# SilentView/EMCID

Hardware: AMD Instinct MI355X
Metric: concept-edits/sec (1 000-concept batch, SD-v1.4) (higher is better)
Workload: dtype f32 forward (2 x fp16 split MFMA, fp32 accumulate) + f64 solve

## Files before the change

emcid_amd/csrc/clip_layers.hip:

```cpp
#include "common.h"

#include <algorithm>

namespace emcid {

__global__ __launch_bounds__(256) void gather_rows16_kernel(const unsigned char* __restrict__ src, int64_t src_stride,
                                                             const int* __restrict__ idx, unsigned char* __restrict__ dst,
                                                             int64_t dst_stride, int row_bytes) {
    typedef unsigned int v4u __attribute__((ext_vector_type(4)));
    const int64_t r = blockIdx.x;
    const v4u* s = reinterpret_cast<const v4u*>(src + (int64_t)idx[r] * src_stride);
    v4u* d = reinterpret_cast<v4u*>(dst + r * dst_stride);
    for (int i = threadIdx.x; i < row_bytes / 16; i += 256) d[i] = s[i];
}

__global__ __launch_bounds__(256) void gather_f32_kernel(const float* __restrict__ src, const int* __restrict__ idx,
                                                          float* __restrict__ dst, int n) {
    const int i = blockIdx.x * 256 + threadIdx.x;
    if (i < n) dst[i] = src[idx[i]];
}

__device__ __forceinline__ unsigned long long fp_mix(unsigned long long x) {
    x ^= x >> 30; x *= 0xBF58476D1CE4E5B9ull; x ^= x >> 27; x *= 0x94D049BB133111EBull; x ^= x >> 31;
    return x;
}

__device__ __forceinline__ unsigned long long fingerprint_of(const unsigned char* data, long long bytes, unsigned long long* lds) {
    typedef unsigned long long v2u64 __attribute__((ext_vector_type(2)));
    const long long nvec = bytes / 16, ns = nvec < 4096 ? nvec : 4096;
    unsigned long long h = 0;
    v2u64 x[16];
#pragma unroll
    for (int u = 0; u < 16; ++u) {
        const long long i = threadIdx.x + 256 * u;
        const long long v = ns == nvec ? i : i * nvec / ns;
        x[u] = i < ns ? *reinterpret_cast<const v2u64*>(data + 16 * v) : (v2u64){0ull, 0ull};
    }
#pragma unroll
    for (int u = 0; u < 16; ++u) {
        const long long i = threadIdx.x + 256 * u;
        if (i < ns)
            h ^= fp_mix(x[u][0] + 0x9E3779B97F4A7C15ull * (unsigned long long)(2 * i + 1)) ^ fp_mix(x[u][1] + 0x9E3779B97F4A7C15ull * (unsigned long long)(2 * i + 2));
    }
#pragma unroll
    for (int o = 32; o > 0; o >>= 1) {
        const unsigned lo = __shfl_xor((unsigned)(h & 0xffffffffu), o, 64), hi = __shfl_xor((unsigned)(h >> 32), o, 64);
        h ^= ((unsigned long long)hi << 32) | lo;
    }
    if ((threadIdx.x & 63) == 0) lds[threadIdx.x >> 6] = h;
    __syncthreads();
    return lds[0] ^ lds[1] ^ lds[2] ^ lds[3];
}

struct FpBatch { const unsigned char* data[32]; long long bytes[32]; long long slot[32]; };

__global__ __launch_bounds__(256) void fingerprint_store_kernel(FpBatch b, long long* table) {
    __shared__ unsigned long long lds[4];
    const unsigned char* data = b.data[blockIdx.x];
    const long long bytes = b.bytes[blockIdx.x];
    const unsigned long long h = fingerprint_of(data, bytes, lds);
    if (threadIdx.x == 0) {
        long long* e = table + 4 * b.slot[blockIdx.x];
        e[0] = (long long)reinterpret_cast<uintptr_t>(data); e[1] = bytes; e[2] = (long long)h; e[3] = 0;
    }
}

__global__ __launch_bounds__(256) void fingerprint_content_kernel(FpBatch b, unsigned long long* out) {
    __shared__ unsigned long long lds[4];
    const unsigned long long h = fingerprint_of(b.data[blockIdx.x], b.bytes[blockIdx.x], lds);
    if (threadIdx.x == 0) out[b.slot[blockIdx.x]] = h;
}

struct FpSkip { unsigned long long m[4]; };

__global__ __launch_bounds__(256) void fingerprint_check_kernel(const long long* table, long long first_slot, FpSkip skip, int* flag) {
    __shared__ unsigned long long lds[4];
    if ((skip.m[blockIdx.x >> 6] >> (blockIdx.x & 63)) & 1ull) return;
    const long long* e = table + 4 * (first_slot + blockIdx.x);
    const long long bytes = e[1];
    if (bytes <= 0) return;
    const unsigned long long h = fingerprint_of(reinterpret_cast<const unsigned char*>((uintptr_t)e[0]), bytes, lds);
    if (threadIdx.x == 0 && h != (unsigned long long)e[2]) atomicOr(flag, 1);
}

struct ClipWs {
    float* qkv;
    float* mid;
    uint32_t* ctx_p;
    float* ctx_s;
    uint32_t* z_p;
    float* z_s;
    float* f_scale;
    uint32_t* f_p;
    uint32_t* xq_p;
    float* xq_s;
    float* hs_q;
};

inline int64_t clip_ws_bytes(int64_t rows, int64_t h, int64_t d) {
    const int64_t r = round_up(rows, 64);
    return 4 * (r * 3 * h + r * h + r * h + r + r * h + r + 2 * r + r * d + r * h + r + r * h) + 16 * 16;
}

inline bool clip_ws_carve(void* base, int64_t bytes, int64_t rows, int64_t h, int64_t d, ClipWs& w) {
    if (base == nullptr || !aligned16(base) || bytes < clip_ws_bytes(rows, h, d)) return false;
    const int64_t r = round_up(rows, 64);
    char* p = (char*)base;
    auto take = [&](int64_t n4) { char* q = p; p += round_up(4 * n4, 16); return q; };
    w.qkv = (float*)take(r * 3 * h);
    w.mid = (float*)take(r * h);
    w.ctx_p = (uint32_t*)take(r * h);
    w.ctx_s = (float*)take(r);
    w.z_p = (uint32_t*)take(r * h);
    w.z_s = (float*)take(r);
    w.f_scale = (float*)take(2 * r);
    w.f_p = (uint32_t*)take(r * d);
    w.xq_p = (uint32_t*)take(r * h);
    w.xq_s = (float*)take(r);
    w.hs_q = (float*)take(r * h);
    return true;
}

}

using namespace emcid;

extern "C" {

int emcid_fingerprint_store(int64_t n, const void* const* data, const int64_t* bytes, const int64_t* slots, void* table,
                            int64_t table_slots, void* stream) {
    EMCID_CHECK_ARG(n >= 0 && table && (n == 0 || (data && bytes && slots)));
    for (int64_t i0 = 0; i0 < n; i0 += 32) {
        FpBatch b{};
        const int cnt = (int)std::min<int64_t>(32, n - i0);
        for (int i = 0; i < cnt; ++i) {
            EMCID_CHECK_ARG(data[i0 + i] && bytes[i0 + i] > 0 && bytes[i0 + i] % 16 == 0 && aligned16(data[i0 + i]) &&
                            slots[i0 + i] >= 0 && slots[i0 + i] < table_slots);
            b.data[i] = (const unsigned char*)data[i0 + i]; b.bytes[i] = bytes[i0 + i]; b.slot[i] = slots[i0 + i];
        }
        hipLaunchKernelGGL(fingerprint_store_kernel, dim3((unsigned)cnt), dim3(256), 0, (hipStream_t)stream, b, (long long*)table);
    }
    EMCID_CHECK_LAUNCH();
    return EMCID_OK;
}

int emcid_fingerprint_check(const void* table, int64_t table_slots, int64_t first_slot, int64_t n_slots, const uint64_t* skip_mask,
                            int* flag, void* stream) {
    EMCID_CHECK_ARG(table && flag && first_slot >= 0 && n_slots >= 0 && first_slot + n_slots <= table_slots && n_slots <= 256);
    if (n_slots == 0) return EMCID_OK;
    FpSkip skip{};
    if (skip_mask != nullptr)
        for (int w = 0; w < 4; ++w) skip.m[w] = skip_mask[w];
    hipLaunchKernelGGL(fingerprint_check_kernel, dim3((unsigned)n_slots), dim3(256), 0, (hipStream_t)stream, (const long long*)table,
                       (long long)first_slot, skip, flag);
    EMCID_CHECK_LAUNCH();
    return EMCID_OK;
}

int emcid_fingerprint_content(int64_t n, const void* const* data, const int64_t* bytes, uint64_t* out_dev, void* stream) {
    EMCID_CHECK_ARG(n >= 0 && (n == 0 || (data && bytes && out_dev)));
    if (n == 0) return EMCID_OK;
    for (int64_t i = 0; i < n; ++i)
        EMCID_CHECK_ARG(data[i] && bytes[i] > 0 && bytes[i] % 16 == 0 && aligned16(data[i]));
    for (int64_t i0 = 0; i0 < n; i0 += 32) {
        FpBatch b{};
        const int cnt = (int)std::min<int64_t>(32, n - i0);
        for (int i = 0; i < cnt; ++i) {
            b.data[i] = (const unsigned char*)data[i0 + i]; b.bytes[i] = bytes[i0 + i]; b.slot[i] = i0 + i;
        }
        hipLaunchKernelGGL(fingerprint_content_kernel, dim3((unsigned)cnt), dim3(256), 0, (hipStream_t)stream, b,
                           (unsigned long long*)out_dev);
    }
    EMCID_CHECK_LAUNCH();
    return EMCID_OK;
}

int64_t emcid_clip_workspace_bytes(int64_t rows, int64_t h, int64_t d) { return clip_ws_bytes(rows, h, d); }

int emcid_clip_layer_head_sp16(const emcid_clip_layer_sp16* L, int64_t rows, int64_t h, int64_t d, int64_t heads, float attn_scale,
                               const int* anc, int64_t anc_ld, const int* depth, const int* rows_sel, int64_t n_sel,
                               const float* hs, const void* x_planes, const float* x_inv_scale, float* mid, void* f_planes,
                               float* f_scale, float* f_f32, void* workspace, int64_t workspace_bytes, void* stream) {
    EMCID_CHECK_ARG(L && rows > 0 && h > 0 && d > 0 && heads > 0 && h % heads == 0 && anc && depth && hs && x_planes && x_inv_scale);
    EMCID_CHECK_ARG(mid && f_planes && f_scale && n_sel > 0 && n_sel <= rows && (rows_sel != nullptr || n_sel == rows) && h % 32 == 0 && d % 32 == 0);
    ClipWs w;
    if (!clip_ws_carve(workspace, workspace_bytes, rows, h, d, w)) return fail(EMCID_ERR_BAD_ARG, __func__, "workspace too small or misaligned");
    hipStream_t st = (hipStream_t)stream;
    const int64_t D = h / heads;
    const float* q;
    int64_t ldq;
    const float* res;
    if (rows_sel == nullptr) {
        EMCID_TRY(emcid_linear_sp16_f32(x_planes, h, x_inv_scale, L->qkv_planes, h, L->qkv_inv_scale, L->qkv_bias, nullptr, 0, w.qkv,
                                        3 * h, nullptr, 0, nullptr, rows, 3 * h, h, 0, -1, stream));
        q = w.qkv, ldq = 3 * h, res = hs;
    } else {
        EMCID_TRY(emcid_linear_sp16_f32(x_planes, h, x_inv_scale, (const uint32_t*)L->qkv_planes + h * h, h, L->qkv_inv_scale + h,
                                        L->qkv_bias ? L->qkv_bias + h : nullptr, nullptr, 0, w.qkv + h, 3 * h, nullptr, 0, nullptr,
                                        rows, 2 * h, h, 0, -1, stream));
        {
            ScopedProf sp(KC_MISC, st);
            hipLaunchKernelGGL(gather_rows16_kernel, dim3((unsigned)n_sel), dim3(256), 0, st, (const unsigned char*)x_planes, 4 * h,
                               rows_sel, (unsigned char*)w.xq_p, 4 * h, (int)(4 * h));
            hipLaunchKernelGGL(gather_f32_kernel, dim3((unsigned)((n_sel + 255) / 256)), dim3(256), 0, st, x_inv_scale, rows_sel,
                               w.xq_s, (int)n_sel);
            hipLaunchKernelGGL(gather_rows16_kernel, dim3((unsigned)n_sel), dim3(256), 0, st, (const unsigned char*)hs, 4 * h,
                               rows_sel, (unsigned char*)w.hs_q, 4 * h, (int)(4 * h));
            EMCID_CHECK_LAUNCH();
        }
        EMCID_TRY(emcid_linear_sp16_f32(w.xq_p, h, w.xq_s, L->qkv_planes, h, L->qkv_inv_scale, L->qkv_bias, nullptr, 0, w.mid, h,
                                        nullptr, 0, nullptr, n_sel, h, h, 0, -1, stream));
        q = w.mid, ldq = h, res = w.hs_q;
    }
    EMCID_TRY(emcid_tree_attention_sp16(q, ldq, w.qkv + h, w.qkv + 2 * h, 3 * h, anc, anc_ld, depth, rows_sel, n_sel, heads, D,
                                        attn_scale, w.ctx_p, h, w.ctx_s, stream));
    EMCID_TRY(emcid_linear_sp16_f32(w.ctx_p, h, w.ctx_s, L->out_planes, h, L->out_inv_scale, L->out_bias, res, h, mid, h, nullptr,
                                    0, nullptr, n_sel, h, h, 0, -1, stream));
    EMCID_TRY(emcid_add_layernorm_sp16(mid, h, nullptr, 0, L->ln2_gamma, L->ln2_beta, L->ln2_eps, n_sel, h, nullptr, nullptr, w.z_p,
                                       h, w.z_s, L->fc1_bound, f_scale, stream));
    EMCID_TRY(emcid_linear_sp16_f32(w.z_p, h, w.z_s, L->fc1_planes, h, L->fc1_inv_scale, L->fc1_bias, nullptr, 0, f_f32, d,
                                    f_planes, d, f_scale, n_sel, d, h, L->act, -1, stream));
    return EMCID_OK;
}

int emcid_clip_layer_tail_sp16(const emcid_clip_layer_sp16* L, int64_t n, int64_t h, int64_t d, const void* f_planes,
                               const float* f_inv_scale, const float* mid, float* hs_out, const float* next_ln_gamma,
                               const float* next_ln_beta, float next_ln_eps, void* x_planes, float* x_inv_scale, void* stream) {
    EMCID_CHECK_ARG(L && n > 0 && h % 32 == 0 && d % 32 == 0 && f_planes && f_inv_scale && mid && hs_out);
    EMCID_TRY(emcid_linear_sp16_f32(f_planes, d, f_inv_scale, L->fc2_planes, d, L->fc2_inv_scale, L->fc2_bias, mid, h, hs_out, h,
                                    nullptr, 0, nullptr, n, h, d, 0, -1, stream));
    if (next_ln_gamma != nullptr) {
        EMCID_CHECK_ARG(next_ln_beta && x_planes && x_inv_scale);
        EMCID_TRY(emcid_add_layernorm_sp16(hs_out, h, nullptr, 0, next_ln_gamma, next_ln_beta, next_ln_eps, n, h, nullptr, nullptr,
                                           x_planes, h, x_inv_scale, nullptr, nullptr, stream));
    }
    return EMCID_OK;
}

int emcid_clip_edit_layer_tail_sp16(const emcid_clip_layer_sp16* L, int64_t n_rows, int64_t h, int64_t d, const float* f_f32,
                                    const void* f_planes, const float* f_inv_scale, const float* mid, const int64_t* lookup,
                                    const int64_t* seg, int64_t B, int64_t N, const float* zs_t, double edit_weight,
                                    int layers_left, double lam_ratio, const void* cov_factor_ws, int64_t n_layers,
                                    int64_t layer_index, int use_inverse, const float* W0, float* W, float* dW, float* K_out,
                                    float* Zc_out, void* k_planes, float* k_inv_scale, void* dual_ws, int64_t dual_ws_bytes,
                                    int* info_dev, void* linear_ws, int64_t linear_ws_bytes, float* hs_out,
                                    const float* next_ln_gamma, const float* next_ln_beta, float next_ln_eps, void* x_planes,
                                    float* x_inv_scale, void* stream) {
    EMCID_CHECK_ARG(L && n_rows > 0 && h % 32 == 0 && d % 32 == 0 && f_f32 && lookup && seg && B > 0 && N > 0 && zs_t);
    EMCID_CHECK_ARG(cov_factor_ws && W0 && W && K_out && Zc_out && dual_ws && info_dev && (hs_out == nullptr || (f_planes && f_inv_scale && mid)));
    EMCID_TRY(emcid_gather_mean_f32(f_f32, B, n_rows, d, 0, d, lookup, seg, N, K_out, d, stream));
    EMCID_CHECK_ARG((k_planes == nullptr) == (k_inv_scale == nullptr));
    if (k_planes != nullptr) {
        EMCID_TRY(emcid_split_rows_f16(K_out, d, N, d, k_planes, d, k_inv_scale, nullptr, stream));
        EMCID_TRY(emcid_linear_sp16_f32(k_planes, d, k_inv_scale, L->fc2_planes, d, L->fc2_inv_scale, L->fc2_bias, nullptr, 0, Zc_out, h,
                                        nullptr, 0, nullptr, N, h, d, 0, -1, stream));
    } else {
        EMCID_TRY(emcid_linear_ws_f32(K_out, d, W, d, L->fc2_bias, nullptr, 0, Zc_out, h, N, h, d, 0, -1, linear_ws, linear_ws_bytes, stream));
    }
    EMCID_TRY(emcid_edit_dual_apply_stage1_f64(K_out, Zc_out, zs_t, N, d, h, edit_weight, layers_left, lam_ratio, cov_factor_ws,
                                               n_layers, layer_index, 0, N, use_inverse, dual_ws, dual_ws_bytes, stream));
    EMCID_TRY(emcid_edit_dual_apply_stage2_f64(N, d, h, cov_factor_ws, n_layers, layer_index, use_inverse, 0, W0, W, dW, dual_ws,
                                               dual_ws_bytes, info_dev, stream));
    if (hs_out != nullptr) {
        EMCID_TRY(emcid_split_rows_f16(W, d, h, d, const_cast<void*>(L->fc2_planes), d, const_cast<float*>(L->fc2_inv_scale), nullptr,
                                       stream));
        EMCID_TRY(emcid_clip_layer_tail_sp16(L, n_rows, h, d, f_planes, f_inv_scale, mid, hs_out, next_ln_gamma, next_ln_beta,
                                             next_ln_eps, x_planes, x_inv_scale, stream));
    }
    return EMCID_OK;
}

int emcid_clip_layers_sp16(const emcid_clip_layer_sp16* layers, int64_t n_layers, int64_t rows, int64_t h, int64_t d, int64_t heads,
                           float attn_scale, const int* anc, int64_t anc_ld, const int* depth, float* hs, void* x_planes,
                           float* x_inv_scale, const float* next_ln_gamma, const float* next_ln_beta, float next_ln_eps,
                           void* workspace, int64_t workspace_bytes, void* stream) {
    EMCID_CHECK_ARG(layers && n_layers > 0 && hs && x_planes && x_inv_scale);
    ClipWs w;
    if (!clip_ws_carve(workspace, workspace_bytes, rows, h, d, w)) return fail(EMCID_ERR_BAD_ARG, __func__, "workspace too small or misaligned");
    for (int64_t i = 0; i < n_layers; ++i) {
        const emcid_clip_layer_sp16* L = layers + i;
        EMCID_TRY(emcid_clip_layer_head_sp16(L, rows, h, d, heads, attn_scale, anc, anc_ld, depth, nullptr, rows, hs, x_planes,
                                             x_inv_scale, w.mid, w.f_p, w.f_scale, nullptr, workspace, workspace_bytes, stream));
        const bool last = i + 1 == n_layers;
        const float* g = last ? next_ln_gamma : layers[i + 1].ln1_gamma;
        const float* b = last ? next_ln_beta : layers[i + 1].ln1_beta;
        const float eps = last ? next_ln_eps : layers[i + 1].ln1_eps;
        EMCID_TRY(emcid_clip_layer_tail_sp16(L, rows, h, d, w.f_p, w.f_scale + rows, w.mid, hs, g, b, eps, x_planes, x_inv_scale, stream));
    }
    return EMCID_OK;
}

}
```

emcid_amd/csrc/gemm_sp16.hip:

```cpp
#include "common.h"
#include "sp16.h"

#include <algorithm>

namespace emcid {

typedef _Float16 v8h __attribute__((ext_vector_type(8)));
typedef _Float16 v4h __attribute__((ext_vector_type(4)));
typedef float v16f __attribute__((ext_vector_type(16)));
typedef float v4f __attribute__((ext_vector_type(4)));
typedef unsigned int v4u __attribute__((ext_vector_type(4)));

#ifndef SP16_ONE_SLOT
#define SP16_ONE_SLOT 0
#endif
constexpr int SPK = 32;

enum SpAct : int { SP_ACT_NONE = 0, SP_ACT_QUICK_GELU = 1, SP_ACT_GELU_ERF = 2 };

template <int V> struct SpIC { static constexpr int value = V; };

__device__ __forceinline__ bool sp_al16(const void* p) { return (reinterpret_cast<uintptr_t>(p) & 15) == 0; }

struct SpArgs {
    const uint32_t* X; int64_t ldx; const float* xs;
    const uint32_t* W; int64_t ldw; const float* ws;
    const float* bias;
    const float* res; int64_t ldr;
    float* Y; int64_t ldy;
    uint32_t* P; int64_t ldp; const float* ps;
    int M, N, K, act, tiles_n, tiles, rb;
    long long* stamps;
};

__device__ __forceinline__ void sp_tile_of(const SpArgs& a, int tile, int& bm, int& bn) {
    const int tiles_m = a.tiles / a.tiles_n, sr = tile / (a.rb * a.tiles_n), rem = tile - sr * a.rb * a.tiles_n;
    const int rows = min(a.rb, tiles_m - sr * a.rb);
    bn = rem / rows;
    bm = sr * a.rb + (rem - bn * rows);
}

template <int MJ, int NI, int WM, int WN, int PF, int KS>
struct SpGeom {
    static constexpr int NW = WM * WN;
    static constexpr int NT = 64 * NW * KS;
    static constexpr int BM = 32 * MJ * WM, BN = 32 * NI * WN;
    static constexpr int PPR = 8 * KS;
    static constexpr int SBK = SPK * KS;
    static constexpr int ROW = 128 * KS + 16;
    static constexpr int VA = (BM * PPR + NT - 1) / NT, VB = (BN * PPR + NT - 1) / NT;
    static constexpr int STAGE = (BM + BN) * ROW;
    static constexpr int NBLK = MJ * NI, HB = KS == 2 ? (NBLK + 1) / 2 : NBLK;
    static constexpr int RED = KS == 2 ? NW * NBLK * 4 * 64 * 16 : 0;
    static constexpr int SMEM = 2 * STAGE > RED ? 2 * STAGE : RED;
};

template <int MJ, int NI, int WM, int WN, int PF, int DBG, int KS>
__device__ __forceinline__ void sp_accumulate(const SpArgs& a, int m0, int n0, int T, unsigned char* smem, v16f (&acc)[NI][MJ]) {
    using G = SpGeom<MJ, NI, WM, WN, PF, KS>;
    constexpr int NT = G::NT, BM = G::BM, BN = G::BN, VA = G::VA, VB = G::VB, STAGE = G::STAGE, PPR = G::PPR, SPROW = G::ROW,
                  SBK = G::SBK;
    const int tid = threadIdx.x, lane = tid & 63, wave = (tid >> 6) % G::NW, grp = (tid >> 6) / G::NW;
    const int l31 = lane & 31, l5 = lane >> 5;
    const int wm0 = (wave / WN) * (32 * MJ), wn0 = (wave % WN) * (32 * NI);

    const uint32_t* pa[VA];
    const uint32_t* pb[VB];
    int wa[VA], wb[VB];
#pragma unroll
    for (int s = 0; s < VA; ++s) {
        const int v = tid + NT * s, row = min(v / PPR, BM - 1);
        pa[s] = a.X + (int64_t)min(m0 + row, a.M - 1) * a.ldx + 4 * (v % PPR);
        wa[s] = row * SPROW + 16 * (v % PPR);
    }
#pragma unroll
    for (int s = 0; s < VB; ++s) {
        const int v = tid + NT * s, row = min(v / PPR, BN - 1);
        pb[s] = a.W + (int64_t)min(n0 + row, a.N - 1) * a.ldw + 4 * (v % PPR);
        wb[s] = (BM + row) * SPROW + 16 * (v % PPR);
    }
    constexpr bool TAIL_A = (BM * PPR) % NT != 0, TAIL_B = (BN * PPR) % NT != 0;
    const bool last_a = !TAIL_A || tid + NT * (VA - 1) < BM * PPR;
    const bool last_b = !TAIL_B || tid + NT * (VB - 1) < BN * PPR;

    v4u ga[PF][VA], gb[PF][VB];
    auto gload = [&](int it, auto rc) __attribute__((always_inline)) {
        constexpr int R = decltype(rc)::value;
        const int k0 = it * SBK;
#pragma unroll
        for (int s = 0; s < VA; ++s)
            if (s + 1 < VA || last_a) ga[R][s] = *reinterpret_cast<const v4u*>(pa[s] + k0);
#pragma unroll
        for (int s = 0; s < VB; ++s)
            if (s + 1 < VB || last_b) gb[R][s] = *reinterpret_cast<const v4u*>(pb[s] + k0);
    };
    auto lstore = [&](unsigned char* stage, auto rc) __attribute__((always_inline)) {
        constexpr int R = decltype(rc)::value;
#pragma unroll
        for (int s = 0; s < VA; ++s)
            if (s + 1 < VA || last_a) *reinterpret_cast<v4u*>(stage + wa[s]) = ga[R][s];
#pragma unroll
        for (int s = 0; s < VB; ++s)
            if (s + 1 < VB || last_b) *reinterpret_cast<v4u*>(stage + wb[s]) = gb[R][s];
    };

    const int fx_off = (wm0 + l31) * SPROW + 32 * l5 + 128 * grp;
    const int fw_off = (BM + wn0 + l31) * SPROW + 32 * l5 + 128 * grp;
    constexpr int NSLOT = ((MJ * NI > 4 && SP16_ONE_SLOT) || MJ * NI > 5) ? 1 : 2;
    v8h xh[NSLOT][MJ], xl[NSLOT][MJ], wh[NSLOT][NI], wl[NSLOT][NI];
    auto fread = [&](const unsigned char* stage, int t, int slot) __attribute__((always_inline)) {
#pragma unroll
        for (int j = 0; j < MJ; ++j) {
            xh[slot][j] = *reinterpret_cast<const v8h*>(stage + fx_off + j * 32 * SPROW + 64 * t);
            xl[slot][j] = *reinterpret_cast<const v8h*>(stage + fx_off + j * 32 * SPROW + 64 * t + 16);
        }
#pragma unroll
        for (int i = 0; i < NI; ++i) {
            wh[slot][i] = *reinterpret_cast<const v8h*>(stage + fw_off + i * 32 * SPROW + 64 * t);
            wl[slot][i] = *reinterpret_cast<const v8h*>(stage + fw_off + i * 32 * SPROW + 64 * t + 16);
        }
    };
    auto mfmas = [&](int slot, int p_lo, int p_hi) __attribute__((always_inline)) {
#pragma unroll
        for (int p = 0; p < 3; ++p)
            if (p >= p_lo && p < p_hi)
#pragma unroll
                for (int i = 0; i < NI; ++i)
#pragma unroll
                    for (int j = 0; j < MJ; ++j)
                        acc[i][j] = __builtin_amdgcn_mfma_f32_32x32x16_f16(p == 0 ? wl[slot][i] : wh[slot][i],
                                                                           p == 1 ? xl[slot][j] : xh[slot][j], acc[i][j], 0, 0, 0);
    };

    gload(0, SpIC<0>{});
    lstore(smem, SpIC<0>{});
    gload(min(1, T - 1), SpIC<1 % PF>{});
    if constexpr (PF > 1) gload(min(2, T - 1), SpIC<2 % PF>{});
    __syncthreads();
    constexpr bool ONE_SLOT = (MJ * NI > 4 && SP16_ONE_SLOT) || MJ * NI > 5;
    if constexpr (!ONE_SLOT) fread(smem, 0, 0);
    if constexpr (DBG >= 3) fread(smem, 1, 1);
    auto body = [&](auto rc, int it) __attribute__((always_inline)) {
        unsigned char* cur = smem + (it & 1) * STAGE;
        unsigned char* oth = smem + ((it + 1) & 1) * STAGE;
        if constexpr (ONE_SLOT) {
            fread(cur, 0, 0);
            mfmas(0, 0, 3);
            __builtin_amdgcn_sched_barrier(0);
            fread(cur, 1, 0);
            lstore(oth, rc);
            __syncthreads();
            gload(min(it + 1 + PF, T - 1), rc);
            __builtin_amdgcn_sched_barrier(0);
            mfmas(0, 0, 3);
            return;
        }
        __builtin_amdgcn_sched_barrier(0);
        mfmas(0, 0, 1);
        __builtin_amdgcn_sched_barrier(0);
        if constexpr (DBG < 3) fread(cur, 1, 1);
        __builtin_amdgcn_sched_barrier(0);
        mfmas(0, 1, 3);
        __builtin_amdgcn_sched_barrier(0);
        if constexpr (DBG < 2) lstore(oth, rc);
        __syncthreads();
        if constexpr (DBG < 1) gload(min(it + 1 + PF, T - 1), rc);
        __builtin_amdgcn_sched_barrier(0);
        mfmas(1, 0, 1);
        __builtin_amdgcn_sched_barrier(0);
        if constexpr (DBG < 3) fread(oth, 0, 0);
        __builtin_amdgcn_sched_barrier(0);
        mfmas(1, 1, 3);
    };
    if constexpr (PF == 1) {
        for (int it = 0; it < T; ++it) body(SpIC<0>{}, it);
    } else {
        int it = 0;
        for (; it + 1 < T; it += 2) {
            body(SpIC<1>{}, it);
            body(SpIC<0>{}, it + 1);
        }
        if (it < T) body(SpIC<1>{}, it);
    }
}

template <int MJ, int NI, int WM, int WN, int KS>
__device__ __forceinline__ void sp_finish(const SpArgs& a, int m0, int n0, unsigned char* smem, v16f (&acc)[NI][MJ]) {
    constexpr int BM = 32 * MJ * WM, BN = 32 * NI * WN, NW = WM * WN, NBLK = MJ * NI, HB = KS == 2 ? (NBLK + 1) / 2 : NBLK;
    const int tid = threadIdx.x, lane = tid & 63, wave = (tid >> 6) % NW, grp = (tid >> 6) / NW;
    const int l31 = lane & 31, l5 = lane >> 5;
    const int wm0 = (wave / WN) * (32 * MJ), wn0 = (wave % WN) * (32 * NI);
    if constexpr (KS == 2) {
        __syncthreads();
        v4f* red = reinterpret_cast<v4f*>(smem) + wave * (NBLK * 4 * 64) + lane;
        auto put = [&](auto tc) __attribute__((always_inline)) {
            constexpr int t = decltype(tc)::value;
#pragma unroll
            for (int q = 0; q < 4; ++q) {
                v4f v = {acc[t / MJ][t % MJ][4 * q], acc[t / MJ][t % MJ][4 * q + 1], acc[t / MJ][t % MJ][4 * q + 2],
                         acc[t / MJ][t % MJ][4 * q + 3]};
                red[(t * 4 + q) * 64] = v;
            }
        };
        auto take = [&](auto tc, auto first) __attribute__((always_inline)) {
            constexpr int t = decltype(tc)::value;
#pragma unroll
            for (int q = 0; q < 4; ++q) {
                const v4f v = red[(t * 4 + q) * 64];
#pragma unroll
                for (int e = 0; e < 4; ++e) {
                    const float c = acc[t / MJ][t % MJ][4 * q + e];
                    acc[t / MJ][t % MJ][4 * q + e] = decltype(first)::value ? c + v[e] : v[e] + c;
                }
            }
        };
        static_assert(NBLK <= 8, "blocks per wave");
        if (grp == 1) {
            if constexpr (0 < HB) put(SpIC<0>{});
            if constexpr (1 < HB) put(SpIC<1>{});
            if constexpr (2 < HB) put(SpIC<2>{});
            if constexpr (3 < HB) put(SpIC<3>{});
        } else {
            if constexpr (0 >= HB && 0 < NBLK) put(SpIC<0>{});
            if constexpr (1 >= HB && 1 < NBLK) put(SpIC<1>{});
            if constexpr (2 >= HB && 2 < NBLK) put(SpIC<2>{});
            if constexpr (3 >= HB && 3 < NBLK) put(SpIC<3>{});
            if constexpr (4 >= HB && 4 < NBLK) put(SpIC<4>{});
            if constexpr (5 >= HB && 5 < NBLK) put(SpIC<5>{});
            if constexpr (6 >= HB && 6 < NBLK) put(SpIC<6>{});
            if constexpr (7 >= HB && 7 < NBLK) put(SpIC<7>{});
        }
        __syncthreads();
        if (grp == 0) {
            if constexpr (0 < HB) take(SpIC<0>{}, SpIC<1>{});
            if constexpr (1 < HB) take(SpIC<1>{}, SpIC<1>{});
            if constexpr (2 < HB) take(SpIC<2>{}, SpIC<1>{});
            if constexpr (3 < HB) take(SpIC<3>{}, SpIC<1>{});
        } else {
            if constexpr (0 >= HB && 0 < NBLK) take(SpIC<0>{}, SpIC<0>{});
            if constexpr (1 >= HB && 1 < NBLK) take(SpIC<1>{}, SpIC<0>{});
            if constexpr (2 >= HB && 2 < NBLK) take(SpIC<2>{}, SpIC<0>{});
            if constexpr (3 >= HB && 3 < NBLK) take(SpIC<3>{}, SpIC<0>{});
            if constexpr (4 >= HB && 4 < NBLK) take(SpIC<4>{}, SpIC<0>{});
            if constexpr (5 >= HB && 5 < NBLK) take(SpIC<5>{}, SpIC<0>{});
            if constexpr (6 >= HB && 6 < NBLK) take(SpIC<6>{}, SpIC<0>{});
            if constexpr (7 >= HB && 7 < NBLK) take(SpIC<7>{}, SpIC<0>{});
        }
    }
    const float* __restrict__ bias = a.bias;
    const float* __restrict__ res = a.res;
    const float* __restrict__ ws = a.ws;
    float* __restrict__ Y = a.Y;
    uint32_t* __restrict__ P = a.P;
    const int M = a.M, N = a.N;
    const int64_t ldr = a.ldr, ldy = a.ldy, ldp = a.ldp;
    const bool vec_ok = (N & 3) == 0 && (Y == nullptr || ((ldy & 3) == 0 && sp_al16(Y))) &&
                        (res == nullptr || ((ldr & 3) == 0 && sp_al16(res))) && (bias == nullptr || sp_al16(bias)) && sp_al16(ws);
    const bool interior = m0 + BM <= M && n0 + BN <= N && vec_ok;
    auto epilogue = [&](auto actfn) __attribute__((always_inline)) {
#pragma unroll
        for (int j = 0; j < MJ; ++j) {
            const int m = m0 + wm0 + 32 * j + l31;
            const bool m_ok = m < M;
            const float sx = a.xs[min(m, M - 1)];
            const float sp = a.ps != nullptr ? a.ps[min(m, M - 1)] : 1.f;
#pragma unroll
            for (int i = 0; i < NI; ++i) {
                if (KS == 2 && ((i * MJ + j) < HB) != (grp == 0)) continue;
                const int nb = n0 + wn0 + 32 * i + 4 * l5;
                if (interior) {
                    v4f rv[4];
                    if (res != nullptr) {
#pragma unroll
                        for (int q = 0; q < 4; ++q) rv[q] = *reinterpret_cast<const v4f*>(res + (int64_t)m * ldr + nb + 8 * q);
                    }
#pragma unroll
                    for (int q = 0; q < 4; ++q) {
                        const int n = nb + 8 * q;
                        const v4f w4 = *reinterpret_cast<const v4f*>(ws + n);
                        v4f b4 = {0.f, 0.f, 0.f, 0.f};
                        if (bias != nullptr) b4 = *reinterpret_cast<const v4f*>(bias + n);
                        v4f v;
#pragma unroll
                        for (int e = 0; e < 4; ++e) {
                            v[e] = actfn(acc[i][j][4 * q + e] * (sx * w4[e]) + b4[e]);
                            if (res != nullptr) v[e] += rv[q][e];
                        }
                        if (Y != nullptr) *reinterpret_cast<v4f*>(Y + (int64_t)m * ldy + n) = v;
                        if (P != nullptr) {
                            v4h h, l;
#pragma unroll
                            for (int e = 0; e < 4; ++e) {
                                const float t = v[e] * sp;
                                h[e] = (_Float16)t;
                                l[e] = (_Float16)(t - (float)h[e]);
                            }
                            unsigned char* dst = reinterpret_cast<unsigned char*>(P + (int64_t)m * ldp) + (n >> 3) * 32 + 8 * l5;
                            *reinterpret_cast<v4h*>(dst) = h;
                            *reinterpret_cast<v4h*>(dst + 16) = l;
                        }
                    }
                } else {
#pragma unroll
                    for (int q = 0; q < 4; ++q)
#pragma unroll
                        for (int e = 0; e < 4; ++e) {
// ... 108 lines not shown
        }
#pragma unroll
        for (int j = 0; j < MJ; ++j) {
            const int m = m0 + wm0 + 16 * j + l15;
            const bool m_ok = m < M;
            const float sx = a.xs[min(m, M - 1)];
            const float sp = a.ps != nullptr ? a.ps[min(m, M - 1)] : 1.f;
#pragma unroll
            for (int i = 0; i < NI; ++i)
#pragma unroll
                for (int e = 0; e < 4; ++e) {
                    const int n = n0 + wn0 + 16 * i + 4 * l4 + e;
                    if (m_ok && n < N) {
                        float v = actfn(acc[i][j][e] * (sx * ws[n]) + (bias != nullptr ? bias[n] : 0.f));
                        if (res != nullptr) v += res[(int64_t)m * ldr + n];
                        if (Y != nullptr) Y[(int64_t)m * ldy + n] = v;
                        if (P != nullptr) {
                            const float t = v * sp;
                            const _Float16 h = (_Float16)t, l = (_Float16)(t - (float)h);
                            _Float16* dst = reinterpret_cast<_Float16*>(reinterpret_cast<unsigned char*>(P + (int64_t)m * ldp) +
                                                                       (n >> 3) * 32) + (n & 7);
                            dst[0] = h;
                            dst[8] = l;
                        }
                    }
                }
        }
    };
    if (a.act == SP_ACT_QUICK_GELU) epilogue([](float x) { return x / (1.0f + __expf(-1.702f * x)); });
    else if (a.act == SP_ACT_GELU_ERF) epilogue([](float x) { return 0.5f * x * (1.0f + erff(x * 0.70710678118654752440f)); });
    else epilogue([](float x) { return x; });
}

struct SpNoPre {
    __device__ __forceinline__ void load() {}
    __device__ __forceinline__ void store() {}
};

template <int MJ, int NI, int WM, int WN, int NSLOT, int DBG, bool ILV, class Pre>
__device__ __forceinline__ void sp_accumulate16(const uint32_t* Xt, int64_t ldx, int mrows, const uint32_t* Wt, int64_t ldw, int nrows, int T,
                                                unsigned char* smem, v4f (&acc)[NI][MJ], Pre& pre, long long (&clk)[2]) {
    constexpr int NWV = WM * WN, BM = 16 * MJ * WM, BN = 16 * NI * WN;
    constexpr int ROWB = 128, RPP = 8, CPR = 8;
    constexpr int STAGE = (BM + BN) * ROWB;
    static_assert(BM % RPP == 0 && BN % RPP == 0, "whole pieces per operand");
    const int tid = threadIdx.x, lane = tid & 63, wave = tid >> 6, l15 = lane & 15, l4 = lane >> 4;
    const int wm0 = (wave / WN) * (16 * MJ), wn0 = (wave % WN) * (16 * NI);

    auto make_rsrc = [](const void* ptr) __attribute__((always_inline)) {
        const uint64_t v = reinterpret_cast<uint64_t>(ptr);
        const uint64_t lo = (uint64_t)(unsigned)__builtin_amdgcn_readfirstlane((int)(v & 0xffffffffu));
        const uint64_t hi = (uint64_t)(unsigned)__builtin_amdgcn_readfirstlane((int)(v >> 32));
        return __builtin_amdgcn_make_buffer_rsrc(reinterpret_cast<void*>(lo | (hi << 32)), 0, 0x7fffffff, 0x00020000);
    };
    const __amdgpu_buffer_rsrc_t rsrc_x = make_rsrc(Xt);
    const __amdgpu_buffer_rsrc_t rsrc_w = make_rsrc(Wt);
    constexpr int NPX = BM / RPP, NPW = BN / RPP, PXW = (NPX + NWV - 1) / NWV, PWW = (NPW + NWV - 1) / NWV;
    const int wave_u = __builtin_amdgcn_readfirstlane(wave);
    unsigned off_x[PXW], off_w[PWW];
#pragma unroll
    for (int s = 0; s < PXW; ++s) {
        const int r = RPP * min(wave + NWV * s, NPX - 1) + lane / CPR;
        off_x[s] = (unsigned)(min(r, mrows - 1) * (int)(4 * ldx) + 16 * ((lane % CPR) ^ sp_key16(r)));
    }
#pragma unroll
    for (int s = 0; s < PWW; ++s) {
        const int r = RPP * min(wave + NWV * s, NPW - 1) + lane / CPR;
        off_w[s] = (unsigned)(min(r, nrows - 1) * (int)(4 * ldw) + 16 * ((lane % CPR) ^ sp_key16(r)));
    }
    auto issue = [&](int it, unsigned char* stage) __attribute__((always_inline)) {
#pragma unroll
        for (int s = 0; s < PXW; ++s)
            if (NPX % NWV == 0 || s + 1 < PXW || wave_u + NWV * s < NPX)
                __builtin_amdgcn_raw_ptr_buffer_load_lds(rsrc_x, (__attribute__((address_space(3))) void*)(stage + (wave_u + NWV * s) * 1024), 16,
                                                         (int)off_x[s], (int)(it * ROWB), 0, 0);
#pragma unroll
        for (int s = 0; s < PWW; ++s)
            if (NPW % NWV == 0 || s + 1 < PWW || wave_u + NWV * s < NPW)
                __builtin_amdgcn_raw_ptr_buffer_load_lds(rsrc_w, (__attribute__((address_space(3))) void*)(stage + (NPX + wave_u + NWV * s) * 1024), 16,
                                                         (int)off_w[s], (int)(it * ROWB), 0, 0);
    };
    const int ch = 16 * ((2 * l4) ^ sp_key16(l15));
    const int fx = (wm0 + l15) * ROWB, fw = (BM + wn0 + l15) * ROWB;
#pragma unroll
    for (int i = 0; i < NI; ++i)
#pragma unroll
        for (int j = 0; j < MJ; ++j)
#pragma unroll
            for (int r = 0; r < 4; ++r) acc[i][j][r] = 0.f;
    v8h xh[NSLOT][MJ], xl[NSLOT][MJ], wh[NSLOT][NI], wl[NSLOT][NI];
    auto fread_x = [&](const unsigned char* stage, int j, auto sc) __attribute__((always_inline)) {
        constexpr int S = decltype(sc)::value;
        xh[S][j] = *reinterpret_cast<const v8h*>(stage + fx + j * 16 * ROWB + ch);
        xl[S][j] = *reinterpret_cast<const v8h*>(stage + fx + j * 16 * ROWB + (ch ^ 16));
    };
    auto fread_w = [&](const unsigned char* stage, int i, auto sc) __attribute__((always_inline)) {
        constexpr int S = decltype(sc)::value;
        wh[S][i] = *reinterpret_cast<const v8h*>(stage + fw + i * 16 * ROWB + ch);
        wl[S][i] = *reinterpret_cast<const v8h*>(stage + fw + i * 16 * ROWB + (ch ^ 16));
    };
    auto fread = [&](const unsigned char* stage, auto sc) __attribute__((always_inline)) {
#pragma unroll
        for (int j = 0; j < MJ; ++j) fread_x(stage, j, sc);
#pragma unroll
        for (int i = 0; i < NI; ++i) fread_w(stage, i, sc);
    };
    auto mfma3 = [&](int i, int j, auto sc) __attribute__((always_inline)) {
        constexpr int S = decltype(sc)::value;
        acc[i][j] = __builtin_amdgcn_mfma_f32_16x16x32_f16(wl[S][i], xh[S][j], acc[i][j], 0, 0, 0);
        acc[i][j] = __builtin_amdgcn_mfma_f32_16x16x32_f16(wh[S][i], xl[S][j], acc[i][j], 0, 0, 0);
        acc[i][j] = __builtin_amdgcn_mfma_f32_16x16x32_f16(wh[S][i], xh[S][j], acc[i][j], 0, 0, 0);
    };
    auto mfmas = [&](auto sc) __attribute__((always_inline)) {
        constexpr int S = decltype(sc)::value;
#pragma unroll
        for (int p = 0; p < 3; ++p)
#pragma unroll
            for (int i = 0; i < NI; ++i)
#pragma unroll
                for (int j = 0; j < MJ; ++j)
                    acc[i][j] = __builtin_amdgcn_mfma_f32_16x16x32_f16(p == 0 ? wl[S][i] : wh[S][i], p == 1 ? xl[S][j] : xh[S][j],
                                                                       acc[i][j], 0, 0, 0);
    };

    issue(0, smem);
    if (T > 1) issue(1, smem + STAGE);
    pre.load();
    __builtin_amdgcn_s_waitcnt(0x0f70);
    pre.store();
    __syncthreads();
    __builtin_amdgcn_sched_barrier(0);
    __builtin_amdgcn_s_waitcnt(0xc07f);
    __builtin_amdgcn_sched_barrier(0);
    fread(smem, SpIC<0>{});
    __builtin_amdgcn_sched_barrier(0);
    __builtin_amdgcn_s_waitcnt(0xc07f);
    __builtin_amdgcn_sched_barrier(0);
    if constexpr (DBG == 2) {
        clk[0] = (long long)__builtin_amdgcn_s_memtime();
        clk[1] = (long long)__builtin_amdgcn_s_memrealtime();
    }
    if constexpr (NSLOT == 2) {
        auto body = [&](int it, auto sc) __attribute__((always_inline)) {
            constexpr int S = decltype(sc)::value;
            unsigned char* cur = smem + (it & 1) * STAGE;
            unsigned char* oth = smem + ((it + 1) & 1) * STAGE;
            __builtin_amdgcn_s_waitcnt(0x0f70);
            __builtin_amdgcn_s_barrier();
            __builtin_amdgcn_sched_barrier(0);
            if (DBG != 1 && DBG != 3 && it + 2 < T) issue(it + 2, cur);
            if (DBG != 3 && it + 1 < T) fread(oth, SpIC<S ^ 1>{});
            __builtin_amdgcn_sched_barrier(0);
            mfmas(sc);
            __builtin_amdgcn_sched_barrier(0);
            __builtin_amdgcn_s_waitcnt(0xc07f);
            __builtin_amdgcn_sched_barrier(0);
        };
        auto body_full = [&](int it, auto sc) __attribute__((always_inline)) {
            constexpr int S = decltype(sc)::value;
            constexpr int NREAD = 2 * (MJ + NI), NMFMA = 3 * MJ * NI, MPG = (2 * MJ * NI) / NREAD < 1 ? 1 : (2 * MJ * NI) / NREAD;
            static_assert(NMFMA >= PXW + PWW + MPG * NREAD, "MFMAs to hide the issue under");
            constexpr int NDMA = PXW + PWW;
            unsigned char* cur = smem + (it & 1) * STAGE;
            unsigned char* oth = smem + ((it + 1) & 1) * STAGE;
            __builtin_amdgcn_s_waitcnt(0x0f70);
            __builtin_amdgcn_s_barrier();
            __builtin_amdgcn_sched_barrier(0);
            if (DBG != 1 && DBG != 3) issue(it + 2, cur);
            if (DBG != 3) fread(oth, SpIC<S ^ 1>{});
            mfmas(sc);
#pragma unroll
            for (int g = 0; g < NDMA; ++g) {
                __builtin_amdgcn_sched_group_barrier(0x008, 1, 0);
                __builtin_amdgcn_sched_group_barrier(0x020, 1, 0);
            }
#pragma unroll
            for (int g = 0; g < NREAD; ++g) {
                __builtin_amdgcn_sched_group_barrier(0x008, MPG, 0);
                __builtin_amdgcn_sched_group_barrier(0x100, 1, 0);
            }
            __builtin_amdgcn_sched_group_barrier(0x008, NMFMA - NDMA - MPG * NREAD, 0);
            __builtin_amdgcn_sched_barrier(0);
            __builtin_amdgcn_s_waitcnt(0xc07f);
            __builtin_amdgcn_sched_barrier(0);
        };
        int it = 0;
        if constexpr (ILV) {
            for (; it + 3 < T; it += 2) {
                body_full(it, SpIC<0>{});
                body_full(it + 1, SpIC<1>{});
            }
        }
        for (; it + 1 < T; it += 2) {
            body(it, SpIC<0>{});
            body(it + 1, SpIC<1>{});
        }
        if (it < T) body(it, SpIC<0>{});
    } else {
        for (int it = 0; it < T; ++it) {
            unsigned char* cur = smem + (it & 1) * STAGE;
            unsigned char* oth = smem + ((it + 1) & 1) * STAGE;
            const bool more = DBG != 3 && it + 1 < T;
#pragma unroll
            for (int j = 0; j < MJ / 2; ++j)
#pragma unroll
                for (int i = 0; i < NI; ++i) mfma3(i, j, SpIC<0>{});
            __builtin_amdgcn_sched_barrier(0);
            __builtin_amdgcn_s_waitcnt(0x0070);
            __builtin_amdgcn_s_barrier();
            __builtin_amdgcn_sched_barrier(0);
            if (DBG != 1 && DBG != 3 && it + 2 < T) issue(it + 2, cur);
            if (more) {
#pragma unroll
                for (int j = 0; j < MJ / 2; ++j) fread_x(oth, j, SpIC<0>{});
            }
            __builtin_amdgcn_sched_barrier(0);
#pragma unroll
            for (int j = MJ / 2; j < MJ - 1; ++j) {
#pragma unroll
                for (int i = 0; i < NI; ++i) mfma3(i, j, SpIC<0>{});
                __builtin_amdgcn_sched_barrier(0);
                if (more) fread_x(oth, j, SpIC<0>{});
                __builtin_amdgcn_sched_barrier(0);
            }
#pragma unroll
            for (int i = 0; i < NI; ++i) {
                mfma3(i, MJ - 1, SpIC<0>{});
                __builtin_amdgcn_sched_barrier(0);
                if (more) fread_w(oth, i, SpIC<0>{});
                __builtin_amdgcn_sched_barrier(0);
            }
            if (more) fread_x(oth, MJ - 1, SpIC<0>{});
            __builtin_amdgcn_sched_barrier(0);
        }
    }
}

template <int BM, int BN, int NT>
struct SpSidePre {
    static constexpr int NSV = (BM + BN + NT - 1) / NT;
    const SpArgs& a;
    int m0, n0;
    float* side;
    float sv0[NSV], sv1[NSV];
    __device__ __forceinline__ void load() {
        const int tid = threadIdx.x;
#pragma unroll
        for (int q = 0; q < NSV; ++q) {
            const int e = tid + q * NT;
            sv0[q] = sv1[q] = 0.f;
            if (e < BM) {
                sv0[q] = a.xs[min(m0 + e, a.M - 1)];
                sv1[q] = a.ps != nullptr ? a.ps[min(m0 + e, a.M - 1)] : 1.f;
            } else if (e < BM + BN) {
                sv0[q] = a.ws[min(n0 + e - BM, a.N - 1)];
                sv1[q] = a.bias != nullptr ? a.bias[min(n0 + e - BM, a.N - 1)] : 0.f;
            }
        }
    }
    __device__ __forceinline__ void store() {
        const int tid = threadIdx.x;
#pragma unroll
        for (int q = 0; q < NSV; ++q) {
            const int e = tid + q * NT;
            if (e < BM) side[e] = sv0[q], side[BM + e] = sv1[q];
            else if (e < BM + BN) side[2 * BM + e - BM] = sv0[q], side[2 * BM + BN + e - BM] = sv1[q];
        }
    }
};

template <int MJ, int NI, int WM, int WN, int NSLOT, int DBG, int WPE = 2, bool ILV = (NSLOT == 2)>
__global__ __launch_bounds__(64 * WM * WN) __attribute__((amdgpu_waves_per_eu(WPE, WPE))) void linear_sp16_dma16_kernel(SpArgs a) {
    constexpr int NWV = WM * WN, BM = 16 * MJ * WM, BN = 16 * NI * WN;
    constexpr int STAGE = (BM + BN) * 128;
    static_assert(2 * STAGE >= NWV * 2048 * NI, "the epilogue's LDS regions");
    constexpr int SIDE = 4 * (2 * BM + 2 * BN);
    __shared__ __attribute__((aligned(1024))) unsigned char smem[2 * STAGE + SIDE];
    const int per = (a.tiles + 7) / 8;
    const int tile = (blockIdx.x & 7) * per + (blockIdx.x >> 3);
    if (tile >= a.tiles || (int)(blockIdx.x >> 3) >= per) return;
    int bm, bn;
    sp_tile_of(a, tile, bm, bn);
    long long t_begin = 0;
    if constexpr (DBG == 2) t_begin = (long long)__builtin_amdgcn_s_memrealtime();
    const int m0 = bm * BM, n0 = bn * BN;
    v4f acc[NI][MJ];
    long long clk[2] = {0, 0};
    SpSidePre<BM, BN, 64 * NWV> pre{a, m0, n0, reinterpret_cast<float*>(smem + 2 * STAGE)};
    sp_accumulate16<MJ, NI, WM, WN, NSLOT, DBG, ILV>(a.X + (int64_t)m0 * a.ldx, a.ldx, a.M - m0, a.W + (int64_t)n0 * a.ldw, a.ldw, a.N - n0,
                                                     a.K / SPK, smem, acc, pre, clk);
    if constexpr (DBG == 2) {
        const long long e_clk = (long long)__builtin_amdgcn_s_memtime(), e_real = (long long)__builtin_amdgcn_s_memrealtime();
        if (a.stamps != nullptr && threadIdx.x == 0) {
            long long* st = a.stamps + 8 * (int64_t)blockIdx.x;
            st[0] = clk[0]; st[1] = e_clk; st[2] = clk[1]; st[3] = e_real; st[4] = t_begin;
        }
    }
    sp_finish16<MJ, NI, WM, WN>(a, m0, n0, smem, reinterpret_cast<const float*>(smem + 2 * STAGE), acc);
    if constexpr (DBG == 2) {
        if (a.stamps != nullptr && threadIdx.x == 0) a.stamps[8 * (int64_t)blockIdx.x + 5] = (long long)__builtin_amdgcn_s_memrealtime();
    }
}

__device__ __forceinline__ void sp_split8(const v4f& a, const v4f& b, float s, v4u& hi, v4u& lo) {
    v8h h, l;
#pragma unroll
    for (int e = 0; e < 8; ++e) {
        const float t = (e < 4 ? a[e] : b[e - 4]) * s;
        h[e] = (_Float16)t;
        l[e] = (_Float16)(t - (float)h[e]);
    }
    hi = *reinterpret_cast<v4u*>(&h);
    lo = *reinterpret_cast<v4u*>(&l);
}

__global__ __launch_bounds__(256) void split_rows_kernel(const float* __restrict__ X, int64_t ldx, int rows, int K,
                                                          uint32_t* __restrict__ P, int64_t ldp, float* __restrict__ inv_scale,
                                                          float* __restrict__ max_row_norm) {
    const int lane = threadIdx.x & 63;
    const int64_t row = (int64_t)blockIdx.x * 4 + (threadIdx.x >> 6);
    if (row >= rows) return;
    const float* x = X + row * ldx;
    const int ng = K / 8;
    float amax = 0.f, ss = 0.f;
    for (int g = lane; g < ng; g += 64) {
        const v4f a = *reinterpret_cast<const v4f*>(x + 8 * g), b = *reinterpret_cast<const v4f*>(x + 8 * g + 4);
#pragma unroll
        for (int e = 0; e < 4; ++e) {
            amax = fmaxf(amax, fmaxf(fabsf(a[e]), fabsf(b[e])));
            ss += a[e] * a[e] + b[e] * b[e];
        }
    }
#pragma unroll
    for (int o = 32; o > 0; o >>= 1) {
        amax = fmaxf(amax, __shfl_xor(amax, o, 64));
        ss += __shfl_xor(ss, o, 64);
    }
    if (max_row_norm != nullptr && lane == 0)
        atomicMax(reinterpret_cast<unsigned int*>(max_row_norm), __float_as_uint(sqrtf(ss) * 1.0001f));
    float s, inv;
    sp_scale_of(amax, s, inv);
    if (lane == 0) inv_scale[row] = inv;
    uint32_t* p = P + row * ldp;
    for (int g = lane; g < ng; g += 64) {
        const v4f a = *reinterpret_cast<const v4f*>(x + 8 * g), b = *reinterpret_cast<const v4f*>(x + 8 * g + 4);
        v4u hi, lo;
        sp_split8(a, b, s, hi, lo);
        *reinterpret_cast<v4u*>(p + 8 * g) = hi;
        *reinterpret_cast<v4u*>(p + 8 * g + 4) = lo;
    }
}

__global__ __launch_bounds__(256) void gram_colmax_kernel(const float* __restrict__ X, int64_t ldx, const float* __restrict__ rw, int t,
                                                           int d, int rows_per_wg, unsigned* __restrict__ cmax) {
    const int c4 = blockIdx.x * 256 + threadIdx.x;
    if (4 * c4 >= d) return;
    const int r0 = blockIdx.y * rows_per_wg, r1 = min(t, r0 + rows_per_wg);
    v4f m = {0.f, 0.f, 0.f, 0.f};
    int r = r0;
    for (; r + 8 <= r1; r += 8) {
        v4f x[8];
        float w[8];
#pragma unroll
        for (int u = 0; u < 8; ++u) {
            x[u] = *reinterpret_cast<const v4f*>(X + (int64_t)(r + u) * ldx + 4 * c4);
            w[u] = rw != nullptr ? rw[r + u] : 1.f;
        }
#pragma unroll
        for (int u = 0; u < 8; ++u)
#pragma unroll
            for (int e = 0; e < 4; ++e) m[e] = fmaxf(m[e], fabsf(x[u][e] * w[u]));
    }
    for (; r < r1; ++r) {
        const v4f x = *reinterpret_cast<const v4f*>(X + (int64_t)r * ldx + 4 * c4);
        const float w = rw != nullptr ? rw[r] : 1.f;
#pragma unroll
        for (int e = 0; e < 4; ++e) m[e] = fmaxf(m[e], fabsf(x[e] * w));
    }
#pragma unroll
    for (int e = 0; e < 4; ++e) atomicMax(cmax + 4 * c4 + e, __float_as_uint(m[e]));
}

__global__ __launch_bounds__(256) void gram_transpose_split_kernel(const float* __restrict__ X, int64_t ldx, const float* __restrict__ rw,
                                                                    int t, int d, const unsigned* __restrict__ cmax,
                                                                    uint32_t* __restrict__ P, int64_t ldp, float* __restrict__ inv_scale) {
    __shared__ float tile[64][65];
    const int t0 = blockIdx.x * 64, d0 = blockIdx.y * 64, tid = threadIdx.x;
    for (int v = tid; v < 64 * 16; v += 256) {
        const int r = v >> 4, c = (v & 15) * 4;
        v4f x = {0.f, 0.f, 0.f, 0.f};
        float w = 1.f;
        if (t0 + r < t && d0 + c < d) {
            x = *reinterpret_cast<const v4f*>(X + (int64_t)(t0 + r) * ldx + d0 + c);
            if (rw != nullptr) w = rw[t0 + r];
        }
#pragma unroll
        for (int e = 0; e < 4; ++e) tile[r][c + e] = x[e] * w;
    }
    __syncthreads();
#pragma unroll
    for (int u = 0; u < 2; ++u) {
        const int w = tid + 256 * u, f = w >> 3, g = w & 7;
        if (d0 + f >= d) continue;
        float s, inv;
        sp_scale_of(__uint_as_float(cmax[d0 + f]), s, inv);
        if (blockIdx.x == 0 && g == 0) inv_scale[d0 + f] = inv;
        v4f a, b;
#pragma unroll
        for (int e = 0; e < 4; ++e) a[e] = tile[8 * g + e][f], b[e] = tile[8 * g + 4 + e][f];
        v4u hi, lo;
        sp_split8(a, b, s, hi, lo);
        uint32_t* dst = P + (int64_t)(d0 + f) * ldp + t0 + 8 * g;
        *reinterpret_cast<v4u*>(dst) = hi;
        *reinterpret_cast<v4u*>(dst + 4) = lo;
    }
}

struct GramSpArgs {
    const uint32_t* XT; int64_t ld; const float* inv; float* G; int64_t ldg; int d, K, tiles_side, ks;
};

__global__ __launch_bounds__(256) __attribute__((amdgpu_waves_per_eu(2, 2))) void gram_sp16_kernel(GramSpArgs g) {
    constexpr int MJ = 4, NI = 4, WM = 2, WN = 2, BT = 128;
    __shared__ __attribute__((aligned(1024))) unsigned char smem[2 * (2 * BT) * 128];
    const int n_lower = g.tiles_side * (g.tiles_side + 1) / 2, items = n_lower * g.ks, per = (items + 7) / 8;
    const int item = (blockIdx.x & 7) * per + (blockIdx.x >> 3);
    if (item >= items || (int)(blockIdx.x >> 3) >= per) return;
    const int tile = item / g.ks, part = item - tile * g.ks;
    int bm = (int)((sqrtf(8.f * (float)tile + 1.f) - 1.f) * 0.5f);
    while (bm * (bm + 1) / 2 > tile) --bm;
    while ((bm + 1) * (bm + 2) / 2 <= tile) ++bm;
    const int bn = tile - bm * (bm + 1) / 2;
    const int T = g.K / SPK, it_lo = (int)((int64_t)part * T / g.ks), it_hi = (int)((int64_t)(part + 1) * T / g.ks);
    if (it_hi <= it_lo) return;
    const int c0 = bn * BT, r0 = bm * BT;
    const uint32_t* base = g.XT + (int64_t)it_lo * SPK;
    v4f acc[NI][MJ];
    long long clk[2];
    SpNoPre pre;
    sp_accumulate16<MJ, NI, WM, WN, 2, 0, true>(base + (int64_t)c0 * g.ld, g.ld, g.d - c0, base + (int64_t)r0 * g.ld, g.ld, g.d - r0,
                                                it_hi - it_lo, smem, acc, pre, clk);
    const int tid = threadIdx.x, lane = tid & 63, wave = tid >> 6, l15 = lane & 15, l4 = lane >> 4;
    const int wm0 = (wave / WN) * (16 * MJ), wn0 = (wave % WN) * (16 * NI);
    float rinv[NI][4];
#pragma unroll
    for (int i = 0; i < NI; ++i)
#pragma unroll
        for (int e = 0; e < 4; ++e) rinv[i][e] = g.inv[min(r0 + wn0 + 16 * i + 4 * l4 + e, g.d - 1)];
#pragma unroll
    for (int j = 0; j < MJ; ++j) {
        const int col = c0 + wm0 + 16 * j + l15;
        const float sc = g.inv[min(col, g.d - 1)];
#pragma unroll
        for (int i = 0; i < NI; ++i)
#pragma unroll
            for (int e = 0; e < 4; ++e) {
                const int row = r0 + wn0 + 16 * i + 4 * l4 + e;
                if (row < g.d && col < g.d) unsafeAtomicAdd(g.G + (int64_t)row * g.ldg + col, acc[i][j][e] * (sc * rinv[i][e]));
            }
    }
}

struct SpCfg { int bm, bn; };
static const SpCfg kSpCfgs[] = {{128, 128}, {80, 128}, {64, 64}, {160, 128}, {64, 64}};
inline long long* g_sp16_stamps = nullptr;

}

using namespace emcid;

extern "C" {

int emcid_split_rows_f16(const float* X, int64_t ldx, int64_t rows, int64_t K, void* planes, int64_t ldp, float* inv_scale,
                         float* max_row_norm, void* stream) {
    EMCID_CHECK_ARG(X && planes && inv_scale && rows > 0 && K > 0 && K % 8 == 0 && ldx >= K && ldp >= K);
    EMCID_CHECK_ARG(ldx % 4 == 0 && ldp % 4 == 0 && aligned16(X) && aligned16(planes) && rows < (1LL << 31) && K < (1 << 24));
    ScopedProf sp(KC_MISC, (hipStream_t)stream);
    hipLaunchKernelGGL(split_rows_kernel, dim3((unsigned)((rows + 3) / 4)), dim3(256), 0, (hipStream_t)stream, X, ldx, (int)rows,
                       (int)K, (uint32_t*)planes, ldp, inv_scale, max_row_norm);
    EMCID_CHECK_LAUNCH();
    return EMCID_OK;
}

int64_t emcid_gram_sp16_workspace_bytes_for(int64_t d, int64_t t) {
    const int64_t tc = round_up(t < 1 ? 1 : (t > 32768 ? 32768 : t), 64);
    return round_up(d, 64) * tc * 4 + 2 * round_up(d, 64) * 4 + 256;
}

int64_t emcid_gram_sp16_workspace_bytes(int64_t d) { return emcid_gram_sp16_workspace_bytes_for(d, 32768); }

int emcid_gram_accumulate_sp16_f32(const float* X, const float* row_weight, int64_t t, int64_t d, int64_t ldx, float* G, int64_t ldg,
                                   void* workspace, int64_t workspace_bytes, void* stream) {
    EMCID_CHECK_ARG(X && G && workspace && t >= 0 && d > 0 && ldx >= d && ldg >= d && d % 4 == 0 && ldx % 4 == 0 && aligned16(X));
    EMCID_CHECK_ARG(workspace_bytes >= emcid_gram_sp16_workspace_bytes_for(d, t) && aligned16(workspace) && d < (1 << 20) && t < (1LL << 31));
    if (t == 0) return EMCID_OK;
    hipStream_t st = (hipStream_t)stream;
    const int64_t dr = round_up(d, 64);
    uint32_t* P = (uint32_t*)workspace;
    const int64_t chunk_cap = round_up(std::min<int64_t>(t, 32768), 64);
    unsigned* cmax = (unsigned*)((char*)workspace + dr * chunk_cap * 4);
    float* inv = (float*)(cmax + dr);
    const int side = (int)((d + 127) / 128), n_lower = side * (side + 1) / 2;
    ScopedProf sp(KC_GRAM, st);
    for (int64_t c0 = 0; c0 < t; c0 += 32768) {
        const int tc = (int)std::min<int64_t>(32768, t - c0), tpad = (int)round_up(tc, 64);
        const float* Xc = X + c0 * ldx;
        const float* rwc = row_weight != nullptr ? row_weight + c0 : nullptr;
        if (hipMemsetAsync(cmax, 0, dr * sizeof(unsigned), st) != hipSuccess) return fail(EMCID_ERR_HIP, __func__, "hipMemsetAsync");
        const int rows_per_wg = 64;
        hipLaunchKernelGGL(gram_colmax_kernel, dim3((unsigned)((d / 4 + 255) / 256), (unsigned)((tc + rows_per_wg - 1) / rows_per_wg)),
                           dim3(256), 0, st, Xc, ldx, rwc, tc, (int)d, rows_per_wg, cmax);
        hipLaunchKernelGGL(gram_transpose_split_kernel, dim3((unsigned)(tpad / 64), (unsigned)(dr / 64)), dim3(256), 0, st, Xc, ldx, rwc,
                           tc, (int)d, cmax, P, (int64_t)tpad, inv);
        const int T = tpad / SPK;
        int ks = 1;
        double best = 0.0;
        for (int k = 1; k <= 16 && T / k >= 16; ++k) {
            const int items = n_lower * k;
            const double fill = (double)items / (512.0 * ((items + 511) / 512));
            const double score = fill - 0.01 * k + (items >= 1024 ? 0.0 : -0.5);
            if (score > best) best = score, ks = k;
        }
        GramSpArgs ga{P, (int64_t)tpad, inv, G, ldg, (int)d, tpad, side, ks};
        const int items = n_lower * ks;
        hipLaunchKernelGGL(gram_sp16_kernel, dim3((unsigned)(((items + 7) / 8) * 8)), dim3(256), 0, st, ga);
    }
    EMCID_CHECK_LAUNCH();
    return EMCID_OK;
}

int emcid_debug_linear_sp16_stamps(long long* stamps_dev) {
    g_sp16_stamps = stamps_dev;
    return EMCID_OK;
}

int emcid_linear_sp16_f32(const void* Xp, int64_t ldx, const float* x_inv_scale, const void* Wp, int64_t ldw,
                          const float* w_inv_scale, const float* bias, const float* residual, int64_t ldr, float* Y, int64_t ldy,
                          void* Yp, int64_t ldp, const float* y_scale, int64_t M, int64_t N, int64_t K, int act, int cfg,
                          void* stream) {
    EMCID_CHECK_ARG(Xp && Wp && x_inv_scale && w_inv_scale && (Y || Yp) && M > 0 && N > 0 && K > 0 && ldx >= K && ldw >= K);
    EMCID_CHECK_ARG(K % SPK == 0 && ldx % 4 == 0 && ldw % 4 == 0 && aligned16(Xp) && aligned16(Wp));
    EMCID_CHECK_ARG(M < (1 << 24) && N < (1 << 24) && K < (1 << 24) && (residual == nullptr || ldr >= N) && (Y == nullptr || ldy >= N));
    EMCID_CHECK_ARG(Yp == nullptr || (N % 8 == 0 && ldp >= N && ldp % 4 == 0 && aligned16(Yp)));
    EMCID_CHECK_ARG(act >= SP_ACT_NONE && act <= SP_ACT_GELU_ERF && cfg >= -1 && cfg < 64);
    EMCID_CHECK_ARG(ldx < (1 << 20) && ldw < (1 << 20));
    const int dbg = cfg < 0 ? 0 : (cfg >> 4) & 3;
    int tile_sel = cfg < 0 ? -1 : (cfg & 15);
    EMCID_CHECK_ARG(tile_sel <= 4 && (dbg == 0 || tile_sel == 0) && dbg != 2);
    if (tile_sel < 0) {
        const int64_t t128 = ((M + 127) / 128) * ((N + 127) / 128), t80 = ((M + 79) / 80) * ((N + 127) / 128);
        const int64_t t64 = ((M + 63) / 64) * ((N + 63) / 64);
        if (t128 >= 1600 && M >= 16384) tile_sel = 3;
        else if (t128 >= 400) tile_sel = 0;
        else if (t80 >= 400) tile_sel = 1;
        else if (t64 >= 256) tile_sel = 2;
        else tile_sel = 4;
    }
    const int bm = kSpCfgs[tile_sel].bm, bn = kSpCfgs[tile_sel].bn;
    const int tiles_m = (int)((M + bm - 1) / bm), tiles_n = (int)((N + bn - 1) / bn);
    const int tiles = tiles_m * tiles_n;
    const int per = (tiles + 7) / 8;
    hipStream_t st = (hipStream_t)stream;
    const int rb = 4;
    const SpArgs a{(const uint32_t*)Xp, ldx, x_inv_scale, (const uint32_t*)Wp, ldw, w_inv_scale, bias, residual, ldr, Y, ldy,
                   (uint32_t*)Yp, ldp, y_scale, (int)M, (int)N, (int)K, act, tiles_n, tiles, rb, g_sp16_stamps};
    ScopedProf sp(KC_LINEAR, st);
#define EMCID_SP_DMA16(MJ_, NI_, WM_, WN_, NS_, WPE_, DBG_)                                                                        \
    hipLaunchKernelGGL((linear_sp16_dma16_kernel<MJ_, NI_, WM_, WN_, NS_, DBG_, WPE_>), dim3((unsigned)(per * 8)), dim3(64 * WM_ * WN_), 0, st, a)
    switch (tile_sel) {
        case 0:
            if (dbg == 1) EMCID_SP_DMA16(4, 4, 2, 2, 2, 2, 1);
            else if (dbg == 3) EMCID_SP_DMA16(4, 4, 2, 2, 2, 2, 3);
            else if (a.stamps) EMCID_SP_DMA16(4, 4, 2, 2, 2, 2, 2);
            else EMCID_SP_DMA16(4, 4, 2, 2, 2, 2, 0);
            break;
        case 1: EMCID_SP_DMA16(5, 2, 1, 4, 2, 2, 0); break;
        case 2: EMCID_SP_DMA16(2, 2, 2, 2, 2, 4, 0); break;
        case 3: EMCID_SP_DMA16(5, 4, 2, 2, 1, 2, 0); break;
        default:
            hipLaunchKernelGGL((linear_sp16_kernel<1, 1, 2, 2, 2, 4, 0, 1>), dim3((unsigned)(per * 8)), dim3(256), 0, st, a);
            break;
    }
#undef EMCID_SP_DMA16
    EMCID_CHECK_LAUNCH();
    return EMCID_OK;
}

}
```

emcid_amd/csrc/sp16.h:

```cpp
#pragma once
#include <hip/hip_runtime.h>
#include <stdint.h>

namespace emcid {

typedef _Float16 sp_v4h __attribute__((ext_vector_type(4)));

__device__ __forceinline__ void sp_scale_of(float amax, float& s, float& inv) {
    int ex = (int)((__float_as_uint(amax) >> 23) & 0xff);
    ex = ex == 0 ? 1 : (ex == 255 ? 254 : ex);
    int e = 141 - ex;
    e = e > 120 ? 120 : (e < -120 ? -120 : e);
    s = __uint_as_float((unsigned)(e + 127) << 23);
    inv = __uint_as_float((unsigned)(127 - e) << 23);
}

__device__ __forceinline__ void sp_store4(uint32_t* row_planes, int col, float x0, float x1, float x2, float x3, float s) {
    sp_v4h h, l;
    const float t0 = x0 * s, t1 = x1 * s, t2 = x2 * s, t3 = x3 * s;
    h[0] = (_Float16)t0; h[1] = (_Float16)t1; h[2] = (_Float16)t2; h[3] = (_Float16)t3;
    l[0] = (_Float16)(t0 - (float)h[0]); l[1] = (_Float16)(t1 - (float)h[1]);
    l[2] = (_Float16)(t2 - (float)h[2]); l[3] = (_Float16)(t3 - (float)h[3]);
    unsigned char* dst = reinterpret_cast<unsigned char*>(row_planes) + (col >> 3) * 32 + ((col >> 2) & 1) * 8;
    *reinterpret_cast<sp_v4h*>(dst) = h;
    *reinterpret_cast<sp_v4h*>(dst + 16) = l;
}

}
```

emcid_amd/hip.py:

```python
from __future__ import annotations

import ctypes as C
import math
import os
import threading
from pathlib import Path
from typing import Optional

import torch

_LIB_PATH = Path(__file__).resolve().parent / "csrc" / "libemcid_hip.so"
_lib = None

EXPORTS = [
    "emcid_abi_version", "emcid_last_error", "emcid_gram_accumulate_f32", "emcid_symmetrize_lower_f32",
    "emcid_gather_mean_f32", "emcid_edit_workspace_bytes", "emcid_edit_layer_f64", "emcid_assemble_spd_f64",
    "emcid_cholesky_f64", "emcid_cholesky_solve_f64", "emcid_delta_w_f64", "emcid_dgemm_f64", "emcid_dgemm_ex_f64", "emcid_dgemm_batched_f64", "emcid_streamk_workspace_bytes", "emcid_dgemm_streamk_f64", "emcid_debug_streamk_stamps", "emcid_debug_step_stamps", "emcid_debug_linear_sp16_stamps", "emcid_fingerprint_store", "emcid_fingerprint_check", "emcid_fingerprint_content", "emcid_axpy_f32",
    "emcid_profile_enable", "emcid_profile_collect", "emcid_attention_f32", "emcid_edit_layer_shard_f64",
    "emcid_apply_update_f32", "emcid_inverse_workspace_doubles", "emcid_quick_gelu_f32", "emcid_add_layernorm_f32", "emcid_embed_layernorm_f32", "emcid_tree_attention_f32", "emcid_debug_leaf_stamps",
    "emcid_cov_factor_workspace_bytes", "emcid_factor_cov_f64", "emcid_cov_inverse_f64", "emcid_cov_factor_rescale_f64",
    "emcid_edit_dual_workspace_bytes",
    "emcid_edit_dual_stage1_f64", "emcid_edit_dual_pt", "emcid_edit_dual_stage2_f64",
    "emcid_edit_dual_apply_stage1_f64", "emcid_edit_dual_yt", "emcid_edit_dual_apply_stage2_f64",
    "emcid_edit_dual_apply_assemble_f64",
    "emcid_edit_dual_preserve_workspace_bytes", "emcid_edit_layer_dual_preserve_f64",
    "emcid_session_retain_workspace_bytes", "emcid_session_retain_f64", "emcid_session_step_norms_f64",
    "emcid_session_release_workspace_bytes", "emcid_session_release_f64",
    "emcid_cov_factor_fold_workspace_bytes", "emcid_cov_factor_fold_f64",
    "emcid_session_refold_update_f64", "emcid_cov_factor_refactor_f64",
    "emcid_score_rows_f32", "emcid_score_chains_f64", "emcid_score_chains_pair_f64", "emcid_score_pooled_f32",
    "emcid_edit_lu_workspace_bytes", "emcid_edit_layer_lu_f64", "emcid_lu_solve_f64",
    "emcid_edit_dual_cols_stage1_f64", "emcid_edit_dual_s", "emcid_edit_dual_u", "emcid_edit_dual_cols_stage2_f64",
    "emcid_apply_update2d_f32", "emcid_linear_f32", "emcid_linear_ws_f32", "emcid_linear_workspace_bytes",
    "emcid_split_rows_f16", "emcid_linear_sp16_f32", "emcid_gram_sp16_workspace_bytes", "emcid_gram_sp16_workspace_bytes_for", "emcid_gram_accumulate_sp16_f32", "emcid_add_layernorm_sp16", "emcid_embed_layernorm_sp16",
    "emcid_tree_attention_sp16", "emcid_tree_attention_sp16_supported", "emcid_clip_workspace_bytes",
    "emcid_clip_layer_head_sp16", "emcid_clip_layer_tail_sp16", "emcid_clip_layers_sp16", "emcid_clip_edit_layer_tail_sp16",
    "emcid_edit_dual_block", "emcid_edit_dual_schur_form", "emcid_full_inverse_scratch_doubles", "emcid_full_inverse_f64",
]
DUAL_BLOCKS = ["K", "P", "Y", "R", "S", "LS", "INVS", "PT", "Y2", "V", "U", "SK", "XT", "TT", "SK_COUNTERS"]
SCHUR_FORMS = ["xrow", "full_inverse", "substitution"]
PROF_CLASSES = ["prep", "assemble", "chol_leaf", "chol_panel", "chol_trail", "trsm_diag", "trsm_update", "delta_w",
                "gram", "gather", "dgemm", "misc", "inv_build", "chol_inner", "inv_apply", "inv_block", "linear"]

ABI_VERSION = 16
NB = 128
NPAD = 64


class EmcidHipError(RuntimeError):
    pass


def lib_path() -> Path:
    return _LIB_PATH


def load():
    global _lib
    if _lib is not None:
        return _lib
    if not _LIB_PATH.exists():
        raise EmcidHipError(
            f"{_LIB_PATH} is missing: build it with `python -c 'import __graft_entry__ as g; g.build()'` "
            f"or `make -C {_LIB_PATH.parent}`. The MI355X path has no CPU fallback.")
    lib = C.CDLL(str(_LIB_PATH))
    p, i64, i32, f64, f32 = C.c_void_p, C.c_int64, C.c_int, C.c_double, C.c_float
    sig = {
        "emcid_abi_version": (i32, []),
        "emcid_last_error": (C.c_char_p, []),
        "emcid_gram_accumulate_f32": (i32, [p, i64, i64, i64, p, i64, i32, p]),
        "emcid_symmetrize_lower_f32": (i32, [p, i64, i64, p]),
        "emcid_gather_mean_f32": (i32, [p, i64, i64, i64, i64, i64, p, p, i64, p, i64, p]),
        "emcid_edit_workspace_bytes": (i64, [i64, i64, i64]),
        "emcid_edit_layer_f64": (i32, [p, p, p, p, i64, i64, i64, f64, f64, i32, p, p, p, p, p, p, i64, p, p]),
        "emcid_edit_layer_shard_f64": (i32, [p, p, p, p, i64, i64, i64, f64, f64, i32, i64, i64, p, p, p, p, i64, p, p]),
        "emcid_apply_update_f32": (i32, [p, p, p, p, i64, p]),
        "emcid_assemble_spd_f64": (i32, [p, i64, p, i64, i64, i64, f64, f32, p, i64, p]),
        "emcid_cholesky_f64": (i32, [p, p, i64, i64, p, p, p]),
        "emcid_inverse_workspace_doubles": (i64, [i64]),
        "emcid_debug_leaf_stamps": (i32, [p, p, p, p, p, p]),
        "emcid_cov_factor_workspace_bytes": (i64, [i64, i64]),
        "emcid_factor_cov_f64": (i32, [p, i64, i64, f64, f64, p, i64, p, p]),
        "emcid_cov_inverse_f64": (i32, [p, i64, i64, i64, i64, p]),
        "emcid_cov_factor_rescale_f64": (i32, [p, p, i64, i64, i64, f64, i32, p]),
        "emcid_edit_dual_workspace_bytes": (i64, [i64, i64, i64]),
        "emcid_edit_dual_stage1_f64": (i32, [p, p, p, i64, i64, i64, f64, i32, f64, p, i64, i64, i64, i64, i32, p, i64, p]),
        "emcid_edit_dual_pt": (p, [p, i64, i64, i64]),
        "emcid_edit_dual_block": (p, [p, i64, i64, i64, i32, C.POINTER(i64)]),
        "emcid_edit_dual_schur_form": (i32, [i64, i64, i64]),
        "emcid_full_inverse_scratch_doubles": (i64, [i64, i64]),
        "emcid_full_inverse_f64": (i32, [p, i64, i64, p, p, p, i64, p]),
        "emcid_edit_dual_stage2_f64": (i32, [i64, i64, i64, f64, p, p, p, p, p, p, i64, p, p]),
        "emcid_edit_dual_apply_stage1_f64": (i32, [p, p, p, i64, i64, i64, f64, i32, f64, p, i64, i64, i64, i64, i32, p, i64, p]),
        "emcid_edit_dual_yt": (p, [p, i64, i64, i64]),
        "emcid_edit_dual_apply_stage2_f64": (i32, [i64, i64, i64, p, i64, i64, i32, i32, p, p, p, p, i64, p, p]),
        "emcid_edit_dual_apply_assemble_f64": (i32, [i64, i64, i64, p, i64, p]),
        "emcid_edit_dual_preserve_workspace_bytes": (i64, [i64, i64, i64, i64]),
        "emcid_edit_layer_dual_preserve_f64": (i32, [p, p, p, i64, i64, i64, f64, i32, f64, p, i64, i64, p, i64, p, i64, p, i64, i64,
                                                     p, p, p, p, p, i64, p, p]),
        "emcid_session_retain_workspace_bytes": (i64, [i64, i64, i64]),
        "emcid_session_retain_f64": (i32, [p, i64, i64, f64, f64, p, i64, i64, p, i64, p, i64, p, i64, i64, p, i64, p, p]),
        "emcid_session_step_norms_f64": (i32, [p, i64, i64, i64, i64, i64, i64, p, p, p, p]),
        "emcid_session_release_workspace_bytes": (i64, [i64, i64, i64]),
        "emcid_session_release_f64": (i32, [p, i64, i64, i64, p, i64, p, i64, p, i64, i64, p, i64, p, p]),
        "emcid_cov_factor_fold_workspace_bytes": (i64, [i64, i64]),
        "emcid_cov_factor_fold_f64": (i32, [p, f64, p, i64, i64, i64, p, f64, f64, i32, p, i64, i64, i64, p, p, i64, p, p]),
        "emcid_session_refold_update_f64": (i32, [p, i64, i64, i64, p, i64, i64, i64, p, i64, i64, p, i64, p, p]),
        "emcid_cov_factor_refactor_f64": (i32, [p, i64, i64, i64, p, p]),
        "emcid_score_rows_f32": (i32, [p, i64, p, i64, p, i64, p, p, f32, i64, i64, p, p]),
        "emcid_score_chains_f64": (i32, [p, i64, p, i64, p, p, i64, p, p]),
        "emcid_score_chains_pair_f64": (i32, [p, i64, p, i64, p, p, p, i64, p, i64, p, p, i64, p, p]),
        "emcid_score_pooled_f32": (i32, [p, i64, p, i64, p, p, f32, p, i64, i64, i64, i64, p, p]),
        "emcid_cholesky_solve_f64": (i32, [p, i64, i64, p, p, p, i64, i64, p]),
        "emcid_edit_dual_cols_stage1_f64": (i32, [p, p, p, i64, i64, i64, f64, i32, f64, p, i64, i64, p, i32, p, i64, p]),
        "emcid_edit_dual_s": (p, [p, i64, i64, i64]),
        "emcid_edit_dual_u": (p, [p, i64, i64, i64]),
        "emcid_edit_dual_cols_stage2_f64": (i32, [i64, i64, i64, p, i64, i64, p, i32, p, i64, p, p]),
        "emcid_apply_update2d_f32": (i32, [p, i64, p, p, p, i64, i64, p]),
        "emcid_edit_lu_workspace_bytes": (i64, [i64, i64, i64]),
        "emcid_edit_layer_lu_f64": (i32, [p, p, p, p, i64, i64, i64, f64, f64, i32, p, p, p, p, p, p, i64, p, p]),
        "emcid_lu_solve_f64": (i32, [p, i64, i64, p, i64, i64, p, p, p]),
        "emcid_delta_w_f64": (i32, [p, i64, p, i64, i64, i64, i64, p, p, i64, p, p, p]),
        "emcid_dgemm_f64": (i32, [i32, i32, i64, i64, i64, f64, p, i64, p, i64, f64, p, i64, p]),
        "emcid_dgemm_ex_f64": (i32, [i32, i32, i64, i64, i64, f64, p, i64, p, i64, f64, p, i64, i32, i32, i32, p]),
        "emcid_dgemm_batched_f64": (i32, [i32, i32, i64, i64, i64, f64, p, i64, i64, p, i64, i64, f64, p, i64, i64, i64, p]),
        "emcid_streamk_workspace_bytes": (i64, [i32]),
        "emcid_debug_streamk_stamps": (i32, [p]),
        "emcid_debug_linear_sp16_stamps": (i32, [p]),
        "emcid_fingerprint_store": (i32, [i64, p, p, p, p, i64, p]),
        "emcid_fingerprint_check": (i32, [p, i64, i64, i64, p, p, p]),
        "emcid_fingerprint_content": (i32, [i64, p, p, p, p]),
        "emcid_debug_step_stamps": (i32, [p]),
        "emcid_dgemm_streamk_f64": (i32, [i32, i64, i64, i64, f64, p, i64, p, i64, p, i64, i32, i32, f64, p, i64, p]),
        "emcid_axpy_f32": (i32, [p, p, i64, p]),
        "emcid_quick_gelu_f32": (i32, [p, p, i64, p]),
        "emcid_linear_f32": (i32, [p, i64, p, i64, p, p, i64, p, i64, i64, i64, i64, i32, i32, p]),
        "emcid_linear_ws_f32": (i32, [p, i64, p, i64, p, p, i64, p, i64, i64, i64, i64, i32, i32, p, i64, p]),
        "emcid_linear_workspace_bytes": (i64, []),
        "emcid_split_rows_f16": (i32, [p, i64, i64, i64, p, i64, p, p, p]),
        "emcid_gram_sp16_workspace_bytes": (i64, [i64]),
        "emcid_gram_sp16_workspace_bytes_for": (i64, [i64, i64]),
        "emcid_gram_accumulate_sp16_f32": (i32, [p, p, i64, i64, i64, p, i64, p, i64, p]),
        "emcid_add_layernorm_sp16": (i32, [p, i64, p, i64, p, p, C.c_float, i64, i64, p, p, p, i64, p, p, p, p]),
        "emcid_embed_layernorm_sp16": (i32, [p, i64, i64, p, i64, i64, p, p, p, p, C.c_float, i64, i64, p, p, p, i64, p, p]),
        "emcid_tree_attention_sp16_supported": (i32, [i64, i64, i64]),
        "emcid_clip_workspace_bytes": (i64, [i64, i64, i64]),
        "emcid_clip_layer_head_sp16": (i32, [p, i64, i64, i64, i64, f32, p, i64, p, p, i64, p, p, p, p, p, p, p, p, i64, p]),
        "emcid_clip_layer_tail_sp16": (i32, [p, i64, i64, i64, p, p, p, p, p, p, f32, p, p, p]),
        "emcid_clip_layers_sp16": (i32, [p, i64, i64, i64, i64, i64, f32, p, i64, p, p, p, p, p, p, f32, p, i64, p]),
        "emcid_clip_edit_layer_tail_sp16": (i32, [p, i64, i64, i64, p, p, p, p, p, p, i64, i64, p, f64, i32, f64, p, i64, i64, i32,
                                                 p, p, p, p, p, p, p, p, i64, p, p, i64, p, p, p, f32, p, p, p]),
        "emcid_tree_attention_sp16": (i32, [p, i64, p, p, i64, p, i64, p, p, i64, i64, i64, f32, p, i64, p, p]),
        "emcid_linear_sp16_f32": (i32, [p, i64, p, p, i64, p, p, p, i64, p, i64, p, i64, p, i64, i64, i64, i32, i32, p]),
        "emcid_add_layernorm_f32": (i32, [p, i64, p, i64, p, p, C.c_float, i64, i64, p, p, p]),
        "emcid_embed_layernorm_f32": (i32, [p, i64, i64, p, i64, i64, p, p, p, p, C.c_float, i64, i64, p, p, p]),
        "emcid_tree_attention_f32": (i32, [p, i64, p, p, i64, p, i64, p, p, i64, i64, i64, f32, p, i64, p]),
        "emcid_profile_enable": (i32, [C.c_uint]),
        "emcid_profile_collect": (i32, [p, p, i32]),
        "emcid_attention_f32": (i32, [p, p, p, i64, i64, i64, p, i32, i64, i64, i32, f32, i64, i64, i64, i64, p, p]),
    }
    for name, (res, args) in sig.items():
        fn = getattr(lib, name)
        fn.restype, fn.argtypes = res, args
    if lib.emcid_abi_version() != ABI_VERSION:
        raise EmcidHipError(f"ABI mismatch: library {lib.emcid_abi_version()} vs binding {ABI_VERSION}; rebuild csrc/")
    _lib = lib
    return lib


_tls = threading.local()


def _check(rc: int, what: str):
    restore = getattr(_tls, "restore", None)
    if restore:
        torch.cuda.set_device(restore.pop())
    if rc != 0:
        raise EmcidHipError(f"{what} failed (rc={rc}): {load().emcid_last_error().decode()}")


def _ptr(t: Optional[torch.Tensor], dtype=None, what="tensor"):
    if t is None:
        return None
    if not t.is_cuda:
        raise EmcidHipError(f"{what} must live in HBM (got device {t.device}); there is no CPU path")
    if dtype is not None and t.dtype != dtype:
        raise EmcidHipError(f"{what} must be {dtype}, got {t.dtype}")
    return C.c_void_p(t.data_ptr())


def _stream(t: torch.Tensor):
    idx = t.device.index
    cur = torch.cuda.current_device()
    if idx is not None and idx != cur:
        if getattr(_tls, "restore", None) is None:
            _tls.restore = []
        _tls.restore.append(cur)
        torch.cuda.set_device(idx)
    return C.c_void_p(torch.cuda.current_stream(t.device).cuda_stream)



GRAM_SPLIT = os.environ.get("EMCID_GRAM_SPLIT", "1") != "0"
_GRAM_WS = {}


def gram_takes_row_weight(X: torch.Tensor, ksplit: int = 0) -> bool:
    d = X.shape[1]
    return bool(GRAM_SPLIT and ksplit != 1 and X.shape[0] >= 2048 and d % 4 == 0 and d >= 256 and X.stride(0) % 4 == 0
                and X.stride(1) == 1 and X.data_ptr() % 16 == 0 and X.dtype == torch.float32)


def gram_accumulate_(G: torch.Tensor, X: torch.Tensor, ksplit: int = 0, row_weight: Optional[torch.Tensor] = None):
    assert X.dim() == 2 and G.dim() == 2 and G.shape[0] == G.shape[1] == X.shape[1]
    assert X.stride(1) == 1 and G.stride(1) == 1
    if X.shape[0] == 0:
        return G
    d = X.shape[1]
    if row_weight is not None:
        assert row_weight.shape == (X.shape[0],) and row_weight.dtype == torch.float32 and row_weight.is_contiguous()
        if not (gram_takes_row_weight(X, ksplit) and G.dtype == torch.float32):
            X, row_weight = X * row_weight.unsqueeze(1), None
    if GRAM_SPLIT and ksplit != 1 and X.shape[0] >= 2048 and d % 4 == 0 and d >= 256 and X.stride(0) % 4 == 0 \
            and X.data_ptr() % 16 == 0 and X.dtype == torch.float32 and G.dtype == torch.float32:
        key = (X.device.index if X.device.index is not None else torch.cuda.current_device(),
               torch.cuda.current_stream(X.device).cuda_stream, d)
        need = int(load().emcid_gram_sp16_workspace_bytes_for(d, X.shape[0]))
        ws = _GRAM_WS.get(key)
        if ws is None or ws.numel() < need:
            if ws is None and len(_GRAM_WS) >= 8:
                _GRAM_WS.clear()
            ws = _GRAM_WS[key] = torch.empty(need, dtype=torch.uint8, device=X.device)
        _check(load().emcid_gram_accumulate_sp16_f32(_ptr(X, torch.float32, "X"),
                                                     _ptr(row_weight, torch.float32, "row_weight") if row_weight is not None else None,
                                                     X.shape[0], d, X.stride(0),
                                                     _ptr(G, torch.float32, "G"), G.stride(0), C.c_void_p(ws.data_ptr()),
                                                     ws.numel(), _stream(G)), "emcid_gram_accumulate_sp16_f32")
        return G
    _check(load().emcid_gram_accumulate_f32(_ptr(X, torch.float32, "X"), X.shape[0], X.shape[1], X.stride(0),
                                            _ptr(G, torch.float32, "G"), G.stride(0), ksplit, _stream(G)),
           "emcid_gram_accumulate_f32")
    return G


def symmetrize_lower_(G: torch.Tensor):
    _check(load().emcid_symmetrize_lower_f32(_ptr(G, torch.float32, "G"), G.shape[0], G.stride(0), _stream(G)),
           "emcid_symmetrize_lower_f32")
    return G



def gather_mean(act: torch.Tensor, idx: torch.Tensor, seg: torch.Tensor, out: Optional[torch.Tensor] = None):
    assert act.dim() == 3 and act.stride(2) == 1
    B, S, c = act.shape
    N = seg.numel() - 1
    assert idx.numel() == B
    if out is None:
        out = torch.empty(N, c, dtype=torch.float32, device=act.device)
    _check(load().emcid_gather_mean_f32(_ptr(act, torch.float32, "act"), B, S, c, act.stride(0), act.stride(1),
                                        _ptr(idx, torch.int64, "idx"), _ptr(seg, torch.int64, "seg"), N,
                                        _ptr(out, torch.float32, "out"), out.stride(0), _stream(act)),
           "emcid_gather_mean_f32")
    return out



def edit_workspace_bytes(N: int, d: int, h: int) -> int:
    return int(load().emcid_edit_workspace_bytes(N, d, h))


class EditWorkspace:

    def __init__(self, N: int, d: int, h: int, device, lu: bool = False):
        self.key = (N, d, h)
        self.lu = lu
        self.nbytes = int(load().emcid_edit_lu_workspace_bytes(N, d, h)) if lu else edit_workspace_bytes(N, d, h)
        self.buf = torch.zeros(self.nbytes // 8, dtype=torch.float64, device=device)
        self.info = torch.zeros(1, dtype=torch.int32, device=device)


def edit_layer(K, Zc, zs_t, Cov, lam: float, edit_weight: float, layers_left: int, W0=None, W=None,
               want_factors: bool = False, want_dw: bool = True, ws: Optional[EditWorkspace] = None):
    N, d = K.shape
    h = Zc.shape[1]
    assert Cov.shape == (d, d) and zs_t.shape == (N, h) and Zc.shape == (N, h)
    for t, nm in ((K, "K"), (Zc, "Zc"), (zs_t, "zs_t"), (Cov, "C")):
        assert t.is_contiguous(), nm
    if ws is None or ws.key != (N, d, h) or ws.lu:
        ws = EditWorkspace(N, d, h, K.device)
    dev = K.device
    Xt = torch.empty(N, d, dtype=torch.float64, device=dev) if want_factors else None
    Rt = torch.empty(N, h, dtype=torch.float64, device=dev) if want_factors else None
    dW = torch.empty(h, d, dtype=torch.float32, device=dev) if want_dw else None
    if W is not None:
        assert W.is_contiguous() and W.shape == (h, d) and W0 is not None and W0.is_contiguous()
    _check(load().emcid_edit_layer_f64(
        _ptr(K, torch.float32, "K"), _ptr(Zc, torch.float32, "Zc"), _ptr(zs_t, torch.float32, "zs_t"),
        _ptr(Cov, torch.float32, "C"), N, d, h, float(lam), float(edit_weight), int(layers_left),
        _ptr(W0, torch.float32, "W0"), _ptr(W, torch.float32, "W"), _ptr(Xt), _ptr(Rt), _ptr(dW),
        _ptr(ws.buf), ws.nbytes, _ptr(ws.info, torch.int32, "info"), _stream(K)), "emcid_edit_layer_f64")
    return {"Xt": Xt, "Rt": Rt, "dW": dW, "ws": ws}


def edit_layer_lu(K, Zc, zs_t, Cov, lam: float, edit_weight: float, layers_left: int, W0=None, W=None,
                  want_factors: bool = False, want_dw: bool = True, ws: Optional[EditWorkspace] = None):
    N, d = K.shape
    h = Zc.shape[1]
    assert Cov.shape == (d, d) and zs_t.shape == (N, h) and Zc.shape == (N, h)
    for t, nm in ((K, "K"), (Zc, "Zc"), (zs_t, "zs_t"), (Cov, "C")):
        assert t.is_contiguous(), nm
    if ws is None or ws.key != (N, d, h) or not ws.lu:
        ws = EditWorkspace(N, d, h, K.device, lu=True)
    dev = K.device
    adj_k = torch.empty(d, N, dtype=torch.float64, device=dev) if want_factors else None
    Rt = torch.empty(N, h, dtype=torch.float64, device=dev) if want_factors else None
    dW = torch.empty(h, d, dtype=torch.float32, device=dev) if want_dw else None
    if W is not None:
        assert W.is_contiguous() and W.shape == (h, d) and W0 is not None and W0.is_contiguous()
    _check(load().emcid_edit_layer_lu_f64(
        _ptr(K, torch.float32, "K"), _ptr(Zc, torch.float32, "Zc"), _ptr(zs_t, torch.float32, "zs_t"),
        _ptr(Cov, torch.float32, "C"), N, d, h, float(lam), float(edit_weight), int(layers_left),
        _ptr(W0, torch.float32, "W0"), _ptr(W, torch.float32, "W"), _ptr(adj_k), _ptr(Rt), _ptr(dW),
        _ptr(ws.buf), ws.nbytes, _ptr(ws.info, torch.int32, "info"), _stream(K)), "emcid_edit_layer_lu_f64")
    return {"adj_k": adj_k, "Rt": Rt, "dW": dW, "ws": ws}


def lu_solve_(A: torch.Tensor, B: torch.Tensor):
    n = A.shape[0]
    piv = torch.zeros(n, dtype=torch.int32, device=A.device)
    info = torch.zeros(1, dtype=torch.int32, device=A.device)
    _check(load().emcid_lu_solve_f64(_ptr(A, torch.float64, "A"), A.stride(0), n, _ptr(B, torch.float64, "B"), B.stride(0),
                                     B.shape[1], _ptr(piv), _ptr(info), _stream(A)), "emcid_lu_solve_f64")
    return piv, info


def edit_layer_shard(K, Zc, zs_t, Cov, lam: float, edit_weight: float, layers_left: int, rows, want_factors=False,
                     ws: Optional[EditWorkspace] = None):
    N, d = K.shape
    h = Zc.shape[1]
    lo, hi = rows
    assert Cov.shape == (d, d) and zs_t.shape == (N, h) and Zc.shape == (N, h) and 0 <= lo < hi <= N
    for t, nm in ((K, "K"), (Zc, "Zc"), (zs_t, "zs_t"), (Cov, "C")):
        assert t.is_contiguous(), nm
    if ws is None or ws.key != (N, d, h) or ws.lu:
        ws = EditWorkspace(N, d, h, K.device)
    dev = K.device
    U = torch.empty(h, d, dtype=torch.float64, device=dev)
    Xt = torch.empty(hi - lo, d, dtype=torch.float64, device=dev) if want_factors else None
    Rt = torch.empty(hi - lo, h, dtype=torch.float64, device=dev) if want_factors else None
    _check(load().emcid_edit_layer_shard_f64(
        _ptr(K, torch.float32, "K"), _ptr(Zc, torch.float32, "Zc"), _ptr(zs_t, torch.float32, "zs_t"),
        _ptr(Cov, torch.float32, "C"), N, d, h, float(lam), float(edit_weight), int(layers_left), lo, hi,
        _ptr(U), _ptr(Xt), _ptr(Rt), _ptr(ws.buf), ws.nbytes, _ptr(ws.info, torch.int32, "info"), _stream(K)),
        "emcid_edit_layer_shard_f64")
    return {"U": U, "Xt": Xt, "Rt": Rt, "ws": ws}


def apply_update_(U, W0, W, want_dw=True):
    assert U.is_contiguous() and W.is_contiguous() and W0.is_contiguous() and U.shape == W.shape
    dW = torch.empty_like(W) if want_dw else None
    _check(load().emcid_apply_update_f32(_ptr(U, torch.float64, "U"), _ptr(W0, torch.float32, "W0"),
                                         _ptr(W, torch.float32, "W"), _ptr(dW), W.numel(), _stream(W)),
           "emcid_apply_update_f32")
    return dW


def dgemm(ta: int, tb: int, A, B, Cm, alpha=1.0, beta=0.0, M=None, N=None, K=None):
    M = M if M is not None else (A.shape[0] if ta == 0 else A.shape[1])
    K = K if K is not None else (A.shape[1] if ta == 0 else A.shape[0])
    N = N if N is not None else (B.shape[0] if tb == 0 else B.shape[1])
    _check(load().emcid_dgemm_f64(ta, tb, M, N, K, float(alpha), _ptr(A, torch.float64), A.stride(0),
                                  _ptr(B, torch.float64), B.stride(0), float(beta), _ptr(Cm, torch.float64),
                                  Cm.stride(0), _stream(Cm)), "emcid_dgemm_f64")
    return Cm


def dgemm_ex(ta: int, tb: int, A, B, Cm, alpha=1.0, beta=0.0, flags=0, cfg=-1, ksplit=0):
    M = A.shape[0] if ta == 0 else A.shape[1]
    K = A.shape[1] if ta == 0 else A.shape[0]
    N = B.shape[0] if tb == 0 else B.shape[1]
    _check(load().emcid_dgemm_ex_f64(ta, tb, M, N, K, float(alpha), _ptr(A, torch.float64), A.stride(0),
                                     _ptr(B, torch.float64), B.stride(0), float(beta), _ptr(Cm, torch.float64),
                                     Cm.stride(0), int(flags), int(cfg), int(ksplit), _stream(Cm)), "emcid_dgemm_ex_f64")
    return Cm


_streamk_ws = {}


def dgemm_streamk(tb: int, A, B, Cm, alpha=1.0, flags=1, wgs=256, diag_add=0.0):
    M, K = A.shape
    N = B.shape[0] if tb == 0 else B.shape[1]
    key = (str(A.device), wgs)
    ws = _streamk_ws.get(key)
    if ws is None:
        ws = _streamk_ws[key] = torch.zeros(int(load().emcid_streamk_workspace_bytes(wgs)) // 8, dtype=torch.float64, device=A.device)
    _check(load().emcid_dgemm_streamk_f64(tb, M, N, K, float(alpha), _ptr(A, torch.float64), A.stride(0), _ptr(B, torch.float64),
                                          B.stride(0), _ptr(Cm, torch.float64), Cm.stride(0), int(flags), int(wgs), float(diag_add),
                                          _ptr(ws), ws.numel() * 8, _stream(Cm)), "emcid_dgemm_streamk_f64")
    return Cm


def dgemm_batched(ta: int, tb: int, A, B, Cm, alpha=1.0, beta=0.0):
    nb = Cm.shape[0]
    M = A.shape[1] if ta == 0 else A.shape[2]
    K = A.shape[2] if ta == 0 else A.shape[1]
    N = B.shape[1] if tb == 0 else B.shape[2]
    for t_, nm in ((A, "A"), (B, "B"), (Cm, "C")):
        if t_.dim() != 3 or t_.stride(2) != 1 or t_.shape[0] != nb:
            raise EmcidHipError(f"dgemm_batched: {nm} must be (batch, rows, cols) with unit inner stride")
    if Cm.shape[1] != M or Cm.shape[2] != N or (B.shape[2] if tb == 0 else B.shape[1]) != K:
        raise EmcidHipError("dgemm_batched: shapes do not agree")
    _check(load().emcid_dgemm_batched_f64(ta, tb, M, N, K, float(alpha), _ptr(A, torch.float64), A.stride(1), A.stride(0),
                                          _ptr(B, torch.float64), B.stride(1), B.stride(0), float(beta),
                                          _ptr(Cm, torch.float64), Cm.stride(1), Cm.stride(0), nb, _stream(Cm)),
           "emcid_dgemm_batched_f64")
    return Cm


def fingerprint_store(entries, table: torch.Tensor):
    n = len(entries)
    if not n:
        return
    ptrs = (C.c_void_p * n)(*[t.data_ptr() for t, _ in entries])
    sizes = (C.c_int64 * n)(*[t.numel() * t.element_size() for t, _ in entries])
    slots = (C.c_int64 * n)(*[int(s) for _, s in entries])
    _check(load().emcid_fingerprint_store(n, ptrs, sizes, slots, _ptr(table, torch.int64, "table"), table.shape[0], _stream(table)),
           "emcid_fingerprint_store")


def fingerprint_check(table: torch.Tensor, first_slot: int, n_slots: int, flag: torch.Tensor, skip=()):
    mask = (C.c_uint64 * 4)()
    for k in skip:
        mask[k >> 6] |= 1 << (k & 63)
    _check(load().emcid_fingerprint_check(_ptr(table, torch.int64, "table"), table.shape[0], int(first_slot), int(n_slots), mask,
                                          _ptr(flag, torch.int32, "flag"), _stream(table)), "emcid_fingerprint_check")


def fingerprint_content(tensors) -> torch.Tensor:
    tensors = list(tensors)
    if not tensors:
        raise EmcidHipError("fingerprint_content needs at least one tensor")
    dev = tensors[0].device
    held = []
    for k, t in enumerate(tensors):
        if not t.is_cuda or t.device != dev:
            raise EmcidHipError(f"fingerprint_content: tensor {k} must live in HBM on {dev} (got {t.device}); there is no CPU path")
        t = t.detach()
        nbytes = t.numel() * t.element_size()
        if nbytes == 0:
            raise EmcidHipError(f"fingerprint_content: tensor {k} is empty")
        if nbytes % 16 or t.data_ptr() % 16 or not t.is_contiguous():
            padded = torch.zeros((nbytes + 15) // 16 * 16, dtype=torch.uint8, device=dev)
            padded[:nbytes].view(t.dtype).copy_(t.reshape(-1))
            t = padded
        held.append(t)
    n = len(held)
    out = torch.zeros(n, dtype=torch.int64, device=dev)
    ptrs = (C.c_void_p * n)(*[t.data_ptr() for t in held])
    sizes = (C.c_int64 * n)(*[t.numel() * t.element_size() for t in held])
    _check(load().emcid_fingerprint_content(n, ptrs, sizes, _ptr(out, torch.int64, "out"), _stream(out)), "emcid_fingerprint_content")
    return out


def axpy_(W: torch.Tensor, dW: torch.Tensor):
    assert W.is_contiguous() and dW.is_contiguous() and W.numel() == dW.numel()
    _check(load().emcid_axpy_f32(_ptr(W, torch.float32, "W"), _ptr(dW, torch.float32, "dW"), W.numel(), _stream(W)),
           "emcid_axpy_f32")
    return W


def cholesky(A: torch.Tensor):
    dp = A.shape[0]
    L = torch.zeros_like(A)
    inv = torch.empty(int(load().emcid_inverse_workspace_doubles(dp)), dtype=torch.float64, device=A.device)
    info = torch.zeros(1, dtype=torch.int32, device=A.device)
    _check(load().emcid_cholesky_f64(_ptr(A, torch.float64), _ptr(L), dp, A.stride(0), _ptr(inv), _ptr(info), _stream(A)),
           "emcid_cholesky_f64")
    return L, inv, info


def cholesky_solve_(L, inv, Bt):
    Y = torch.empty_like(Bt)
    _check(load().emcid_cholesky_solve_f64(_ptr(L, torch.float64), L.shape[0], L.stride(0), _ptr(inv), _ptr(Bt), _ptr(Y),
                                           Bt.shape[0], Bt.stride(0), _stream(Bt)), "emcid_cholesky_solve_f64")
    return Bt


def delta_w_(Rt, Xt, W0, W):
    N, h = Rt.shape
    d = Xt.shape[1]
    assert Xt.shape[0] == N and W.shape == (h, d) and W0.shape == (h, d)
    for t, nm in ((Rt, "Rt"), (Xt, "Xt"), (W0, "W0"), (W, "W")):
        assert t.is_contiguous(), nm
    if h % 2 or d % 2:
        raise EmcidHipError("delta_w_: h and d must be even (16-byte aligned f64 rows)")
    _check(load().emcid_delta_w_f64(_ptr(Rt, torch.float64, "Rt"), h, _ptr(Xt, torch.float64, "Xt"), d, N, h, d,
                                    _ptr(W0, torch.float32, "W0"), _ptr(W, torch.float32, "W"), d, None, None, _stream(W)),
           "emcid_delta_w_f64")
    return W


def profile_enable(classes=()):
    mask = 0
    for c in classes:
        mask |= 1 << PROF_CLASSES.index(c)
    _check(load().emcid_profile_enable(mask), "emcid_profile_enable")


def profile_collect():
    n = len(PROF_CLASSES)
    ms = (C.c_double * n)()
    cnt = (C.c_int64 * n)()
    _check(load().emcid_profile_collect(ms, cnt, n), "emcid_profile_collect")
    return {PROF_CLASSES[i]: (ms[i], int(cnt[i])) for i in range(n) if cnt[i]}


def attention(q, k, v, mask=None, causal=False, scale=None):
    B, H, S, D = q.shape
    for t in (q, k, v):
        if t.stride(3) != 1 or t.stride() != q.stride() or t.shape != q.shape:
            raise EmcidHipError("attention: q/k/v must share shape/strides with unit stride over head_dim")
    out = torch.empty(B, S, H, D, dtype=torch.float32, device=q.device)
    kind, mptr, mb, mi = 0, None, 0, 0
    if mask is not None:
        if mask.dim() != 4 or mask.shape[1] != 1 or mask.shape[2] != S or mask.shape[3] != S or mask.stride(3) != 1:
            mask = mask.expand(-1, 1, S, S).contiguous() if mask.dim() == 4 and mask.shape[1] == 1 else None
            if mask is None:
                raise EmcidHipError("attention: mask must be (B|1, 1, S, S)")
        if mask.dtype == torch.bool:
            kind, mptr = 1, _ptr(mask)
        elif mask.dtype == torch.float32:
            kind, mptr = 2, _ptr(mask)
        else:
            raise EmcidHipError(f"attention: mask dtype {mask.dtype} not supported")
        mb = mask.stride(0) if mask.shape[0] > 1 else 0
        mi = mask.stride(2)
    scale = float(D ** -0.5 if scale is None else scale)
    _check(load().emcid_attention_f32(_ptr(q, torch.float32, "q"), _ptr(k, torch.float32, "k"), _ptr(v, torch.float32, "v"),
                                      q.stride(0), q.stride(1), q.stride(2), mptr, kind, mb, mi, int(bool(causal)), scale,
                                      B, H, S, D, _ptr(out), _stream(q)), "emcid_attention_f32")
    return out


def quick_gelu(x: torch.Tensor) -> torch.Tensor:
    x = x.contiguous()
    y = torch.empty_like(x)
    _check(load().emcid_quick_gelu_f32(_ptr(x, torch.float32, "x"), _ptr(y), x.numel(), _stream(x)), "emcid_quick_gelu_f32")
    return y


ACT_NONE, ACT_QUICK_GELU, ACT_GELU_ERF = 0, 1, 2
LINEAR_FLOPS = {"count": False, "flops": 0.0, "launches": 0}


def linear_supported(x: torch.Tensor, w: torch.Tensor) -> bool:
    return (x.is_cuda and w.is_cuda and x.dtype == torch.float32 and w.dtype == torch.float32 and x.dim() == 2 and w.dim() == 2
            and x.shape[1] == w.shape[1] and x.shape[1] % 16 == 0 and x.stride(1) == 1 and w.stride(1) == 1
            and x.stride(0) % 4 == 0 and w.stride(0) % 4 == 0 and x.data_ptr() % 16 == 0 and w.data_ptr() % 16 == 0
            and x.shape[0] > 0)


_LINEAR_WS = {}


def linear_split_cfg(parts: int, prefetch: int = 2) -> int:
    return 64 + 1 + 4 * (prefetch - 1) + (int(parts) << 7)


def _linear_workspace(dev: torch.device) -> torch.Tensor:
    key = (dev.index if dev.index is not None else torch.cuda.current_device(), torch.cuda.current_stream(dev).cuda_stream)
    ws = _LINEAR_WS.get(key)
    if ws is None:
        if len(_LINEAR_WS) >= 8:
            _LINEAR_WS.clear()
        ws = _LINEAR_WS[key] = torch.zeros(int(load().emcid_linear_workspace_bytes()), dtype=torch.uint8, device=dev)
    return ws


def linear(x: torch.Tensor, w: torch.Tensor, bias: Optional[torch.Tensor] = None, act: int = ACT_NONE,
           residual: Optional[torch.Tensor] = None, out: Optional[torch.Tensor] = None, cfg: int = -1) -> torch.Tensor:
    if not linear_supported(x, w):
        raise EmcidHipError("linear: fp32 HBM operands with K contiguous, K % 16 == 0 and 16-byte aligned rows")
    M, K = x.shape
    N = w.shape[0]
    if out is None:
        out = torch.empty(M, N, dtype=torch.float32, device=x.device)
    if out.shape != (M, N) or out.stride(1) != 1 or out.dtype != torch.float32:
        raise EmcidHipError("linear: out must be an (M, N) fp32 row view")
    if bias is not None and (bias.shape != (N,) or not bias.is_contiguous()):
        raise EmcidHipError("linear: bias must be a contiguous (N,) vector")
    if residual is not None and (residual.shape != (M, N) or residual.stride(1) != 1):
        raise EmcidHipError("linear: residual must be an (M, N) row view")
    if LINEAR_FLOPS["count"]:
        LINEAR_FLOPS["flops"] += 2.0 * M * N * K
        LINEAR_FLOPS["launches"] += 1
    ws = None
    if (cfg >= 128 or (cfg < 0 and K >= 2048 and -(-M // 128) * -(-N // 128) <= 128)) and not torch.cuda.is_current_stream_capturing():
        ws = _linear_workspace(x.device)
    try:
        _check(load().emcid_linear_ws_f32(_ptr(x, torch.float32, "x"), x.stride(0), _ptr(w, torch.float32, "w"), w.stride(0),
                                          _ptr(bias, torch.float32, "bias"), _ptr(residual, torch.float32, "residual"),
                                          residual.stride(0) if residual is not None else 0, _ptr(out, torch.float32, "out"),
                                          out.stride(0), M, N, K, int(act), int(cfg),
                                          C.c_void_p(ws.data_ptr()) if ws is not None else None, ws.numel() if ws is not None else 0,
                                          _stream(x)), "emcid_linear_ws_f32")
    except EmcidHipError:
        if ws is not None:
            _LINEAR_WS.pop((x.device.index if x.device.index is not None else torch.cuda.current_device(),
                            torch.cuda.current_stream(x.device).cuda_stream), None)
        raise
    return out


class SplitRows:
    __slots__ = ("planes", "inv_scale", "f32", "bound", "out_scale")

    def __init__(self, planes: torch.Tensor, inv_scale: torch.Tensor, f32: Optional[torch.Tensor] = None,
                 bound: Optional[torch.Tensor] = None, out_scale: Optional[torch.Tensor] = None):
        self.planes, self.inv_scale, self.f32, self.bound = planes, inv_scale, f32, bound
        self.out_scale = out_scale

    @property
    def shape(self):
        return self.planes.shape

    def index_select(self, idx: torch.Tensor) -> "SplitRows":
        return SplitRows(self.planes.index_select(0, idx), self.inv_scale.index_select(0, idx),
                         self.f32.index_select(0, idx) if self.f32 is not None else None)

    def rows(self, lo: int, hi: int) -> "SplitRows":
        return SplitRows(self.planes[lo:hi], self.inv_scale[lo:hi], self.f32[lo:hi] if self.f32 is not None else None)

    def float(self) -> torch.Tensor:
        if self.f32 is not None:
            return self.f32
        r, k = self.planes.shape
        h = self.planes.contiguous().view(torch.float16).view(r, k // 8, 2, 8).float()
        return ((h[:, :, 0] + h[:, :, 1]).reshape(r, k)) * self.inv_scale[:, None]


def split_supported(x: torch.Tensor) -> bool:
    return (x.is_cuda and x.dtype == torch.float32 and x.dim() == 2 and x.shape[1] % 32 == 0 and x.stride(1) == 1
            and x.stride(0) % 4 == 0 and x.data_ptr() % 16 == 0 and x.shape[0] > 0)


def split_rows(x: torch.Tensor, bias: Optional[torch.Tensor] = None, want_bound: bool = False) -> SplitRows:
    if not split_supported(x):
        raise EmcidHipError("split_rows: fp32 HBM rows with K contiguous, K % 32 == 0 and 16-byte aligned rows")
    rows, K = x.shape
    planes = torch.empty(rows, K, dtype=torch.int32, device=x.device)
    inv = torch.empty(rows, dtype=torch.float32, device=x.device)
    bound = None
    if want_bound:
        bound = torch.zeros(2, dtype=torch.float32, device=x.device)
        if bias is not None:
            bound[1:2] = bias.detach().abs().max()
    _check(load().emcid_split_rows_f16(_ptr(x, torch.float32, "x"), x.stride(0), rows, K, _ptr(planes), planes.stride(0), _ptr(inv),
                                       _ptr(bound), _stream(x)), "emcid_split_rows_f16")
    return SplitRows(planes, inv, None, bound)


def linear_sp(x: SplitRows, w: SplitRows, bias: Optional[torch.Tensor] = None, act: int = ACT_NONE,
              residual: Optional[torch.Tensor] = None, out: Optional[torch.Tensor] = None, want_f32: bool = True,
              planes_scale: Optional[torch.Tensor] = None, cfg: int = -1):
    M, K = x.planes.shape
    N = w.planes.shape[0]
    if w.planes.shape[1] != K or K % 32:
        raise EmcidHipError("linear_sp: operands (M, K) and (N, K) with K % 32 == 0")
    for t in (x.planes, w.planes):
        if t.stride(1) != 1 or t.stride(0) % 4 or t.data_ptr() % 16 or t.dtype != torch.int32:
            raise EmcidHipError("linear_sp: planes must be int32 row views with 16-byte aligned rows")
    dev = x.planes.device
    y = None
    if want_f32 or planes_scale is None:
        y = out if out is not None else torch.empty(M, N, dtype=torch.float32, device=dev)
        if y.shape != (M, N) or y.stride(1) != 1 or y.dtype != torch.float32:
            raise EmcidHipError("linear_sp: out must be an (M, N) fp32 row view")
    yp = None
    if planes_scale is not None:
        if N % 32 or planes_scale.shape != (2, M) or not planes_scale.is_contiguous():
            raise EmcidHipError("linear_sp: planes output needs N % 32 == 0 and a contiguous (2, M) scale / inverse scale")
        yp = torch.empty(M, N, dtype=torch.int32, device=dev)
    if bias is not None and (bias.shape != (N,) or not bias.is_contiguous()):
        raise EmcidHipError("linear_sp: bias must be a contiguous (N,) vector")
    if residual is not None and (residual.shape != (M, N) or residual.stride(1) != 1):
        raise EmcidHipError("linear_sp: residual must be an (M, N) row view")
    if LINEAR_FLOPS["count"]:
        LINEAR_FLOPS["flops"] += 2.0 * M * N * K
        LINEAR_FLOPS["launches"] += 1
    _check(load().emcid_linear_sp16_f32(
        _ptr(x.planes), x.planes.stride(0), _ptr(x.inv_scale, torch.float32, "x scale"), _ptr(w.planes), w.planes.stride(0),
        _ptr(w.inv_scale, torch.float32, "w scale"), _ptr(bias, torch.float32, "bias"), _ptr(residual, torch.float32, "residual"),
        residual.stride(0) if residual is not None else 0, _ptr(y), y.stride(0) if y is not None else 0, _ptr(yp),
        yp.stride(0) if yp is not None else 0, _ptr(planes_scale, torch.float32, "planes scale"), M, N, K, int(act), int(cfg),
        _stream(x.planes)), "emcid_linear_sp16_f32")
    if planes_scale is None:
        return y
    return SplitRows(yp, planes_scale[1], y)


def add_layernorm(a: torch.Tensor, b: Optional[torch.Tensor], ln: torch.nn.LayerNorm, want_sum: bool = True):
    rows, cols = a.shape
    if a.stride(1) != 1 or (b is not None and (b.stride(1) != 1 or b.shape != a.shape)):
        raise EmcidHipError("add_layernorm: (rows, cols) operands with unit column stride")
    if ln.weight is None or ln.bias is None or tuple(ln.normalized_shape) != (cols,):
        raise EmcidHipError("add_layernorm: LayerNorm over the last dimension with affine parameters")
    y = torch.empty(rows, cols, dtype=torch.float32, device=a.device) if (b is not None and want_sum) else None
    z = torch.empty(rows, cols, dtype=torch.float32, device=a.device)
    _check(load().emcid_add_layernorm_f32(_ptr(a, torch.float32, "a"), a.stride(0), _ptr(b, torch.float32, "b"),
                                          b.stride(0) if b is not None else 0,
                                          _ptr(ln.weight, torch.float32, "gamma"), _ptr(ln.bias, torch.float32, "beta"),
                                          float(ln.eps), rows, cols, _ptr(y), _ptr(z), _stream(a)), "emcid_add_layernorm_f32")
    return (a if b is None else y), z


def add_layernorm_sp(a: torch.Tensor, b: Optional[torch.Tensor], ln: torch.nn.LayerNorm, want_sum: bool = True,
                     want_f32: bool = False, bound: Optional[torch.Tensor] = None):
    rows, cols = a.shape
    if a.stride(1) != 1 or (b is not None and (b.stride(1) != 1 or b.shape != a.shape)):
        raise EmcidHipError("add_layernorm_sp: (rows, cols) operands with unit column stride")
    if ln.weight is None or ln.bias is None or tuple(ln.normalized_shape) != (cols,) or cols % 32 or cols > 2048:
        raise EmcidHipError("add_layernorm_sp: LayerNorm over the last dimension with affine parameters, cols % 32 == 0, <= 2048")
    dev = a.device
    y = torch.empty(rows, cols, dtype=torch.float32, device=dev) if (b is not None and want_sum) else None
    z = torch.empty(rows, cols, dtype=torch.float32, device=dev) if want_f32 else None
    planes = torch.empty(rows, cols, dtype=torch.int32, device=dev)
    inv = torch.empty(rows, dtype=torch.float32, device=dev)
    out_scale = torch.empty(2, rows, dtype=torch.float32, device=dev) if bound is not None else None
    _check(load().emcid_add_layernorm_sp16(_ptr(a, torch.float32, "a"), a.stride(0), _ptr(b, torch.float32, "b"),
                                           b.stride(0) if b is not None else 0,
                                           _ptr(ln.weight, torch.float32, "gamma"), _ptr(ln.bias, torch.float32, "beta"),
                                           float(ln.eps), rows, cols, _ptr(y), _ptr(z), _ptr(planes), planes.stride(0), _ptr(inv),
                                           _ptr(bound, torch.float32, "bound"), _ptr(out_scale), _stream(a)),
           "emcid_add_layernorm_sp16")
    return (a if b is None else y), SplitRows(planes, inv, z, None, out_scale)


def embed_layernorm_sp(tok_emb: torch.Tensor, pos_emb: torch.Tensor, token: torch.Tensor, position: torch.Tensor,
                       ln: torch.nn.LayerNorm):
    rows, cols = token.numel(), tok_emb.shape[1]
    if tok_emb.stride(1) != 1 or pos_emb.stride(1) != 1 or pos_emb.shape[1] != cols or position.numel() != rows:
        raise EmcidHipError("embed_layernorm_sp: embedding tables with unit column stride and one index pair per row")
    if ln.weight is None or ln.bias is None or tuple(ln.normalized_shape) != (cols,) or cols % 32 or cols > 2048:
        raise EmcidHipError("embed_layernorm_sp: LayerNorm over the last dimension with affine parameters, cols % 32 == 0, <= 2048")
    y = torch.empty(rows, cols, dtype=torch.float32, device=tok_emb.device)
    planes = torch.empty(rows, cols, dtype=torch.int32, device=tok_emb.device)
    inv = torch.empty(rows, dtype=torch.float32, device=tok_emb.device)
    _check(load().emcid_embed_layernorm_sp16(_ptr(tok_emb, torch.float32, "tok_emb"), tok_emb.stride(0), tok_emb.shape[0],
                                             _ptr(pos_emb, torch.float32, "pos_emb"), pos_emb.stride(0), pos_emb.shape[0],
                                             _ptr(token, torch.int64, "token"), _ptr(position, torch.int32, "position"),
                                             _ptr(ln.weight, torch.float32, "gamma"), _ptr(ln.bias, torch.float32, "beta"),
                                             float(ln.eps), rows, cols, _ptr(y), None, _ptr(planes), planes.stride(0), _ptr(inv),
                                             _stream(tok_emb)), "emcid_embed_layernorm_sp16")
    return y, SplitRows(planes, inv)


def tree_attention_sp_supported(anc: torch.Tensor, H: int, D: int) -> bool:
    return bool(load().emcid_tree_attention_sp16_supported(anc.shape[1], H, D)) and (H * D) % 32 == 0


def tree_attention_sp(q, k, v, anc, depth, H: int, scale=None, rows=None) -> SplitRows:
    U, HD = k.shape
    D = HD // H
    for t in (q, k, v):
        if t.stride(1) != 1 or t.shape[1] != HD:
            raise EmcidHipError("tree_attention_sp: q/k/v must be row-major")
    if k.stride(0) != v.stride(0):
        raise EmcidHipError("tree_attention_sp: k and v must share a leading dimension")
    n = U if rows is None else rows.numel()
    if q.shape[0] != n:
        raise EmcidHipError(f"tree_attention_sp: {q.shape[0]} query rows for {n} query nodes")
    planes = torch.empty(n, HD, dtype=torch.int32, device=q.device)
    inv = torch.empty(n, dtype=torch.float32, device=q.device)
    scale = float(D ** -0.5 if scale is None else scale)
    _check(load().emcid_tree_attention_sp16(
        _ptr(q, torch.float32, "q"), q.stride(0), _ptr(k, torch.float32, "k"), _ptr(v, torch.float32, "v"), k.stride(0),
        _ptr(anc, torch.int32, "anc"), anc.stride(0), _ptr(depth, torch.int32, "depth"),
        _ptr(rows, torch.int32, "rows") if rows is not None else None, n, H, D, scale, _ptr(planes), planes.stride(0), _ptr(inv),
        _stream(q)), "emcid_tree_attention_sp16")
    return SplitRows(planes, inv)


def embed_layernorm(tok_emb: torch.Tensor, pos_emb: torch.Tensor, token: torch.Tensor, position: torch.Tensor,
                    ln: torch.nn.LayerNorm):
    rows, cols = token.numel(), tok_emb.shape[1]
    if tok_emb.stride(1) != 1 or pos_emb.stride(1) != 1 or pos_emb.shape[1] != cols or position.numel() != rows:
        raise EmcidHipError("embed_layernorm: embedding tables with unit column stride and one index pair per row")
    if ln.weight is None or ln.bias is None or tuple(ln.normalized_shape) != (cols,):
        raise EmcidHipError("embed_layernorm: LayerNorm over the last dimension with affine parameters")
    y = torch.empty(rows, cols, dtype=torch.float32, device=tok_emb.device)
    z = torch.empty_like(y)
    _check(load().emcid_embed_layernorm_f32(_ptr(tok_emb, torch.float32, "tok_emb"), tok_emb.stride(0), tok_emb.shape[0],
                                            _ptr(pos_emb, torch.float32, "pos_emb"), pos_emb.stride(0), pos_emb.shape[0],
                                            _ptr(token, torch.int64, "token"), _ptr(position, torch.int32, "position"),
                                            _ptr(ln.weight, torch.float32, "gamma"), _ptr(ln.bias, torch.float32, "beta"),
                                            float(ln.eps), rows, cols, _ptr(y), _ptr(z), _stream(tok_emb)),
           "emcid_embed_layernorm_f32")
    return y, z


def tree_attention(q, k, v, anc, depth, H: int, scale=None, rows=None):
    U, HD = k.shape
    D = HD // H
    for t in (q, k, v):
        if t.stride(1) != 1 or t.shape[1] != HD:
            raise EmcidHipError("tree_attention: q/k/v must be row-major")
    if k.stride(0) != v.stride(0):
        raise EmcidHipError("tree_attention: k and v must share a leading dimension")
    n = U if rows is None else rows.numel()
    if q.shape[0] != n:
        raise EmcidHipError(f"tree_attention: {q.shape[0]} query rows for {n} query nodes")
    out = torch.empty(n, HD, dtype=torch.float32, device=q.device)
    scale = float(D ** -0.5 if scale is None else scale)
    _check(load().emcid_tree_attention_f32(
        _ptr(q, torch.float32, "q"), q.stride(0), _ptr(k, torch.float32, "k"), _ptr(v, torch.float32, "v"), k.stride(0),
        _ptr(anc, torch.int32, "anc"), anc.stride(0), _ptr(depth, torch.int32, "depth"),
        _ptr(rows, torch.int32, "rows") if rows is not None else None, n, H, D, scale, _ptr(out), out.stride(0),
        _stream(q)), "emcid_tree_attention_f32")
    return out



class ClipLayerSp16(C.Structure):
    _fields_ = [(n, C.c_void_p) for n in (
        "ln1_gamma", "ln1_beta", "ln2_gamma", "ln2_beta", "qkv_planes", "qkv_inv_scale", "qkv_bias", "out_planes",
        "out_inv_scale", "out_bias", "fc1_planes", "fc1_inv_scale", "fc1_bias", "fc1_bound", "fc2_planes", "fc2_inv_scale",
        "fc2_bias")] + [("ln1_eps", C.c_float), ("ln2_eps", C.c_float), ("act", C.c_int32), ("reserved", C.c_int32)]


_CLIP_WS = {}


def clip_workspace(dev: torch.device, rows: int, h: int, d: int) -> torch.Tensor:
    key = (dev.index if dev.index is not None else torch.cuda.current_device(), torch.cuda.current_stream(dev).cuda_stream,
           rows, h, d)
    ws = _CLIP_WS.get(key)
    if ws is None:
        if len(_CLIP_WS) >= 16:
            _CLIP_WS.clear()
        ws = _CLIP_WS[key] = torch.empty(int(load().emcid_clip_workspace_bytes(rows, h, d)), dtype=torch.uint8, device=dev)
    return ws


def clip_layers(layer_array, first: int, count: int, rows: int, h: int, d: int, heads: int, scale: float, anc: torch.Tensor,
                depth: torch.Tensor, hs: torch.Tensor, x: "SplitRows", next_ln: Optional[torch.nn.LayerNorm]):
    ws = clip_workspace(hs.device, rows, h, d)
    if LINEAR_FLOPS["count"]:
        LINEAR_FLOPS["flops"] += count * 2.0 * rows * h * (4 * h + 2 * d)
        LINEAR_FLOPS["launches"] += 4 * count
    base = C.addressof(layer_array) + first * C.sizeof(ClipLayerSp16)
    g = _ptr(next_ln.weight, torch.float32, "gamma") if next_ln is not None else None
    b = _ptr(next_ln.bias, torch.float32, "beta") if next_ln is not None else None
    _check(load().emcid_clip_layers_sp16(C.c_void_p(base), count, rows, h, d, heads, float(scale), _ptr(anc, torch.int32, "anc"),
                                         anc.stride(0), _ptr(depth, torch.int32, "depth"), _ptr(hs, torch.float32, "hs"),
                                         _ptr(x.planes), _ptr(x.inv_scale), g, b, float(next_ln.eps) if next_ln is not None else 0.0,
                                         C.c_void_p(ws.data_ptr()), ws.numel(), _stream(hs)), "emcid_clip_layers_sp16")


def clip_layer_head(layer_array, index: int, rows: int, h: int, d: int, heads: int, scale: float, anc: torch.Tensor,
                    depth: torch.Tensor, rows_sel: Optional[torch.Tensor], hs: torch.Tensor, x: "SplitRows", want_f32: bool):
    dev = hs.device
    n = rows if rows_sel is None else rows_sel.numel()
    ws = clip_workspace(dev, rows, h, d)
    mid = torch.empty(n, h, dtype=torch.float32, device=dev)
    f_planes = torch.empty(n, d, dtype=torch.int32, device=dev)
    f_scale = torch.empty(2, n, dtype=torch.float32, device=dev)
    f_f32 = torch.empty(n, d, dtype=torch.float32, device=dev) if want_f32 else None
    if LINEAR_FLOPS["count"]:
        LINEAR_FLOPS["flops"] += 2.0 * h * (rows * (3 * h if rows_sel is None else 2 * h) + n * (h if rows_sel is not None else 0)
                                            + n * h + n * d)
        LINEAR_FLOPS["launches"] += 3 if rows_sel is None else 4
    base = C.addressof(layer_array) + index * C.sizeof(ClipLayerSp16)
    _check(load().emcid_clip_layer_head_sp16(
        C.c_void_p(base), rows, h, d, heads, float(scale), _ptr(anc, torch.int32, "anc"), anc.stride(0),
        _ptr(depth, torch.int32, "depth"), _ptr(rows_sel, torch.int32, "rows") if rows_sel is not None else None, n,
        _ptr(hs, torch.float32, "hs"), _ptr(x.planes), _ptr(x.inv_scale), _ptr(mid), _ptr(f_planes), _ptr(f_scale), _ptr(f_f32),
        C.c_void_p(ws.data_ptr()), ws.numel(), _stream(hs)), "emcid_clip_layer_head_sp16")
    return mid, SplitRows(f_planes, f_scale[1], f_f32)


def clip_layer_tail(layer_array, index: int, h: int, d: int, f: "SplitRows", mid: torch.Tensor,
                    next_ln: Optional[torch.nn.LayerNorm]):
    dev = mid.device
    n = mid.shape[0]
    hs = torch.empty(n, h, dtype=torch.float32, device=dev)
    x = None
    if next_ln is not None:
        x = SplitRows(torch.empty(n, h, dtype=torch.int32, device=dev), torch.empty(n, dtype=torch.float32, device=dev))
    if LINEAR_FLOPS["count"]:
        LINEAR_FLOPS["flops"] += 2.0 * n * h * d
        LINEAR_FLOPS["launches"] += 1
    base = C.addressof(layer_array) + index * C.sizeof(ClipLayerSp16)
    _check(load().emcid_clip_layer_tail_sp16(
        C.c_void_p(base), n, h, d, _ptr(f.planes), _ptr(f.inv_scale), _ptr(mid, torch.float32, "mid"), _ptr(hs),
        _ptr(next_ln.weight, torch.float32, "gamma") if next_ln is not None else None,
        _ptr(next_ln.bias, torch.float32, "beta") if next_ln is not None else None,
        float(next_ln.eps) if next_ln is not None else 0.0, _ptr(x.planes) if x is not None else None,
        _ptr(x.inv_scale) if x is not None else None, _stream(mid)), "emcid_clip_layer_tail_sp16")
    return hs, x


def clip_edit_layer_tail(layer_array, index: int, h: int, d: int, f: "SplitRows", mid: torch.Tensor, lookup: torch.Tensor,
                         seg: torch.Tensor, zs_t: torch.Tensor, factors: "CovFactors", layer_index: int, edit_weight: float,
                         layers_left: int, W0: torch.Tensor, W: torch.Tensor, ws: "DualWorkspace", lam: Optional[float],
                         next_ln: Optional[torch.nn.LayerNorm], last: bool, want_dw: bool = True, zc_split: bool = True):
    dev = mid.device
    n = f.f32.shape[0]
    N = seg.numel() - 1
    K = torch.empty(N, d, dtype=torch.float32, device=dev)
    Zc = torch.empty(N, h, dtype=torch.float32, device=dev)
    dW = torch.empty(h, d, dtype=torch.float32, device=dev) if want_dw else None
    kp = torch.empty(N, d, dtype=torch.int32, device=dev) if zc_split else None
    ks = torch.empty(N, dtype=torch.float32, device=dev) if zc_split else None
    hs = x = None
    if not last:
        hs = torch.empty(n, h, dtype=torch.float32, device=dev)
        if next_ln is not None:
            x = SplitRows(torch.empty(n, h, dtype=torch.int32, device=dev), torch.empty(n, dtype=torch.float32, device=dev))
    lws = _linear_workspace(dev) if (d >= 2048 and -(-N // 128) * -(-h // 128) <= 128
                                     and not torch.cuda.is_current_stream_capturing()) else None
    if LINEAR_FLOPS["count"]:
        LINEAR_FLOPS["flops"] += 2.0 * N * h * d + (0.0 if last else 2.0 * n * h * d)
        LINEAR_FLOPS["launches"] += 1 if last else 2
    base = C.addressof(layer_array) + index * C.sizeof(ClipLayerSp16)
    use_inverse = layer_index in factors.have_inverse
    _check(load().emcid_clip_edit_layer_tail_sp16(
        C.c_void_p(base), n, h, d, _ptr(f.f32, torch.float32, "fc2 input"), _ptr(f.planes), _ptr(f.inv_scale),
        _ptr(mid, torch.float32, "mid"), _ptr(lookup, torch.int64, "lookup"), _ptr(seg, torch.int64, "seg"), lookup.numel(), N,
        _ptr(zs_t, torch.float32, "zs_t"), float(edit_weight), int(layers_left), factors.lam_ratio(lam), _ptr(factors.buf),
        factors.n_layers, int(layer_index), int(bool(use_inverse)), _ptr(W0, torch.float32, "W0"), _ptr(W, torch.float32, "W"),
        _ptr(dW), _ptr(K), _ptr(Zc), _ptr(kp), _ptr(ks), _ptr(ws.buf), ws.nbytes, _ptr(ws.info, torch.int32),
        C.c_void_p(lws.data_ptr()) if lws is not None else None, lws.numel() if lws is not None else 0, _ptr(hs),
        _ptr(next_ln.weight, torch.float32, "gamma") if (next_ln is not None and not last) else None,
        _ptr(next_ln.bias, torch.float32, "beta") if (next_ln is not None and not last) else None,
        float(next_ln.eps) if (next_ln is not None and not last) else 0.0, _ptr(x.planes) if x is not None else None,
        _ptr(x.inv_scale) if x is not None else None, _stream(mid)), "emcid_clip_edit_layer_tail_sp16")
    return {"K": K, "Zc": Zc, "dW": dW, "hs": hs, "x": x}



class CovFactors:

    def __init__(self, n_layers: int, d: int, device):
        self.n_layers, self.d = n_layers, d
        self.nbytes = int(load().emcid_cov_factor_workspace_bytes(n_layers, d))
        self.buf = torch.zeros(self.nbytes // 8, dtype=torch.float64, device=device)
        self.info = torch.zeros(1, dtype=torch.int32, device=device)
        self.dp = (d + NB - 1) // NB * NB
        self._inv = ((self.dp + 511) // 512) * (512 * 512 + 256 * 256)
        self.have_inverse = set()
        self.ready = None
        self.cached = False
        self.lam = None
        self.edit_weight = None

    def lam_ratio(self, lam: Optional[float]) -> float:
        if lam is None or self.lam is None or float(lam) == self.lam:
            return 1.0
        if not (lam > 0.0 and self.lam > 0.0):
            raise EmcidHipError(f"mom2_update_weight must be positive for the Cholesky path (got {lam})")
        return float(lam) / float(self.lam)

    def L(self, layer: int) -> torch.Tensor:
        o = (self.n_layers + layer) * self.dp * self.dp
        return self.buf[o:o + self.dp * self.dp].view(self.dp, self.dp)

    def X(self, layer: int) -> torch.Tensor:
        o = self.n_layers * (2 * self.dp * self.dp + self._inv) + layer * self.dp * self.dp
        return self.buf[o:o + self.dp * self.dp].view(self.dp, self.dp)


def cov_inverse(factors: "CovFactors", first: int = 0, count: Optional[int] = None):
    count = factors.n_layers - first if count is None else count
    _check(load().emcid_cov_inverse_f64(_ptr(factors.buf), factors.n_layers, factors.d, int(first), int(count),
                                        _stream(factors.buf)), "emcid_cov_inverse_f64")
    factors.have_inverse.update(range(first, first + count))


def factor_cov(covs, lam: float, edit_weight: float, factors: Optional[CovFactors] = None, inverse: bool = True) -> CovFactors:
    d = covs[0].shape[0]
    for c in covs:
        assert c.shape == (d, d) and c.is_contiguous()
    if factors is None or factors.n_layers != len(covs) or factors.d != d:
        factors = CovFactors(len(covs), d, covs[0].device)
    arr = (C.c_void_p * len(covs))(*[_ptr(c, torch.float32, "C").value for c in covs])
    _check(load().emcid_factor_cov_f64(arr, len(covs), d, float(lam), float(edit_weight), _ptr(factors.buf), factors.nbytes,
                                       _ptr(factors.info, torch.int32), _stream(covs[0])), "emcid_factor_cov_f64")
    factors.have_inverse = set()
    factors.lam, factors.edit_weight = float(lam), float(edit_weight)
    if inverse:
        cov_inverse(factors)
    return factors


def cov_factor_rescale(src: CovFactors, a: float, dst: Optional[CovFactors] = None, lam: Optional[float] = None,
                       edit_weight: Optional[float] = None) -> CovFactors:
    if not (a > 0.0 and a < 1e300):
        raise EmcidHipError(f"the scale of a factored workspace must be positive and finite (got {a})")
    with_inverse = len(src.have_inverse) == src.n_layers
    if dst is None or dst.n_layers != src.n_layers or dst.d != src.d or dst.buf.device != src.buf.device:
        dst = CovFactors(src.n_layers, src.d, src.buf.device)
# ... 621 lines not shown
```

include/emcid_hip.h:

```cpp
#ifndef EMCID_HIP_H
#define EMCID_HIP_H

#include <stdint.h>

#ifdef __cplusplus
extern "C" {
#endif

#define EMCID_OK 0
#define EMCID_ERR_BAD_ARG (-1)
#define EMCID_ERR_HIP (-2)
#define EMCID_ERR_WORKSPACE (-3)

#define EMCID_ABI_VERSION 16

int emcid_abi_version(void);
const char* emcid_last_error(void);

#define EMCID_PROF_CLASSES 16
int emcid_profile_enable(unsigned class_mask);
int emcid_profile_collect(double* ms_per_class_host, int64_t* launches_per_class_host, int n_classes);

int emcid_gram_accumulate_f32(const float* X, int64_t t, int64_t d, int64_t ldx,
                              float* G, int64_t ldg, int ksplit, void* stream);
int emcid_symmetrize_lower_f32(float* G, int64_t d, int64_t ldg, void* stream);

int emcid_gather_mean_f32(const float* act, int64_t B, int64_t S, int64_t c, int64_t ldb, int64_t lds_,
                          const int64_t* idx, const int64_t* seg, int64_t N,
                          float* out, int64_t ldo, void* stream);

int emcid_attention_f32(const float* q, const float* k, const float* v, int64_t sb, int64_t sh, int64_t ss,
                        const void* mask, int mask_kind, int64_t mb, int64_t mi, int causal, float scale,
                        int64_t B, int64_t H, int64_t S, int64_t D, float* out, void* stream);

int emcid_tree_attention_f32(const float* q, int64_t ldq, const float* k, const float* v, int64_t ld, const int* anc, int64_t anc_ld,
                             const int* depth, const int* rows, int64_t n_rows, int64_t H, int64_t D, float scale,
                             float* out, int64_t ldo, void* stream);

int emcid_quick_gelu_f32(const float* x, float* y, int64_t n, void* stream);

int emcid_linear_f32(const float* X, int64_t ldx, const float* W, int64_t ldw, const float* bias, const float* residual,
                     int64_t ldr, float* Y, int64_t ldy, int64_t M, int64_t N, int64_t K, int act, int cfg, void* stream);

int64_t emcid_linear_workspace_bytes(void);
int emcid_linear_ws_f32(const float* X, int64_t ldx, const float* W, int64_t ldw, const float* bias, const float* residual,
                        int64_t ldr, float* Y, int64_t ldy, int64_t M, int64_t N, int64_t K, int act, int cfg, void* workspace,
                        int64_t workspace_bytes, void* stream);

int emcid_split_rows_f16(const float* X, int64_t ldx, int64_t rows, int64_t K, void* planes, int64_t ldp, float* inv_scale,
                         float* max_row_norm, void* stream);

int emcid_linear_sp16_f32(const void* Xp, int64_t ldx, const float* x_inv_scale, const void* Wp, int64_t ldw,
                          const float* w_inv_scale, const float* bias, const float* residual, int64_t ldr, float* Y, int64_t ldy,
                          void* Yp, int64_t ldp, const float* y_scale, int64_t M, int64_t N, int64_t K, int act, int cfg,
                          void* stream);

int emcid_debug_linear_sp16_stamps(long long* stamps_dev);
int64_t emcid_gram_sp16_workspace_bytes(int64_t d);
int64_t emcid_gram_sp16_workspace_bytes_for(int64_t d, int64_t t);
int emcid_gram_accumulate_sp16_f32(const float* X, const float* row_weight, int64_t t, int64_t d, int64_t ldx, float* G, int64_t ldg,
                                   void* workspace, int64_t workspace_bytes, void* stream);

int emcid_add_layernorm_sp16(const float* a, int64_t lda, const float* b, int64_t ldb, const float* gamma, const float* beta,
                             float eps, int64_t rows, int64_t cols, float* y, float* z, void* planes, int64_t ldp,
                             float* inv_scale, const float* bound, float* out_scale, void* stream);
int emcid_embed_layernorm_sp16(const float* tok, int64_t ld_tok, int64_t n_tok, const float* pos, int64_t ld_pos, int64_t n_pos,
                               const int64_t* token, const int* position, const float* gamma, const float* beta, float eps,
                               int64_t rows, int64_t cols, float* y, float* z, void* planes, int64_t ldp, float* inv_scale,
                               void* stream);
int emcid_tree_attention_sp16_supported(int64_t anc_ld, int64_t H, int64_t D);
int emcid_tree_attention_sp16(const float* q, int64_t ldq, const float* k, const float* v, int64_t ld, const int* anc,
                              int64_t anc_ld, const int* depth, const int* rows, int64_t n_rows, int64_t H, int64_t D, float scale,
                              void* planes, int64_t ldp, float* inv_scale, void* stream);

int emcid_fingerprint_store(int64_t n, const void* const* data, const int64_t* bytes, const int64_t* slots, void* table,
                            int64_t table_slots, void* stream);
int emcid_fingerprint_check(const void* table, int64_t table_slots, int64_t first_slot, int64_t n_slots, const uint64_t* skip_mask,
                            int* flag, void* stream);

int emcid_fingerprint_content(int64_t n, const void* const* data, const int64_t* bytes, uint64_t* out_dev, void* stream);

typedef struct emcid_clip_layer_sp16 {
    const float* ln1_gamma; const float* ln1_beta;
    const float* ln2_gamma; const float* ln2_beta;
    const void* qkv_planes; const float* qkv_inv_scale; const float* qkv_bias;
    const void* out_planes; const float* out_inv_scale; const float* out_bias;
    const void* fc1_planes; const float* fc1_inv_scale; const float* fc1_bias; const float* fc1_bound;
    const void* fc2_planes; const float* fc2_inv_scale; const float* fc2_bias;
    float ln1_eps, ln2_eps;
    int32_t act, reserved;
} emcid_clip_layer_sp16;

int64_t emcid_clip_workspace_bytes(int64_t rows, int64_t h, int64_t d);

int emcid_clip_layer_head_sp16(const emcid_clip_layer_sp16* L, int64_t rows, int64_t h, int64_t d, int64_t heads, float attn_scale,
                               const int* anc, int64_t anc_ld, const int* depth, const int* rows_sel, int64_t n_sel,
                               const float* hs, const void* x_planes, const float* x_inv_scale, float* mid, void* f_planes,
                               float* f_scale, float* f_f32, void* workspace, int64_t workspace_bytes, void* stream);

int emcid_clip_layer_tail_sp16(const emcid_clip_layer_sp16* L, int64_t n, int64_t h, int64_t d, const void* f_planes,
                               const float* f_inv_scale, const float* mid, float* hs_out, const float* next_ln_gamma,
                               const float* next_ln_beta, float next_ln_eps, void* x_planes, float* x_inv_scale, void* stream);

int emcid_clip_edit_layer_tail_sp16(const emcid_clip_layer_sp16* L, int64_t n_rows, int64_t h, int64_t d, const float* f_f32,
                                    const void* f_planes, const float* f_inv_scale, const float* mid, const int64_t* lookup,
                                    const int64_t* seg, int64_t B, int64_t N, const float* zs_t, double edit_weight,
                                    int layers_left, double lam_ratio, const void* cov_factor_ws, int64_t n_layers,
                                    int64_t layer_index, int use_inverse, const float* W0, float* W, float* dW, float* K_out,
                                    float* Zc_out, void* k_planes, float* k_inv_scale, void* dual_ws, int64_t dual_ws_bytes,
                                    int* info_dev, void* linear_ws, int64_t linear_ws_bytes, float* hs_out,
                                    const float* next_ln_gamma, const float* next_ln_beta, float next_ln_eps, void* x_planes,
                                    float* x_inv_scale, void* stream);

int emcid_clip_layers_sp16(const emcid_clip_layer_sp16* layers, int64_t n_layers, int64_t rows, int64_t h, int64_t d, int64_t heads,
                           float attn_scale, const int* anc, int64_t anc_ld, const int* depth, float* hs, void* x_planes,
                           float* x_inv_scale, const float* next_ln_gamma, const float* next_ln_beta, float next_ln_eps,
                           void* workspace, int64_t workspace_bytes, void* stream);

int emcid_add_layernorm_f32(const float* a, int64_t lda, const float* b, int64_t ldb, const float* gamma, const float* beta,
                            float eps, int64_t rows, int64_t cols, float* y, float* z, void* stream);

int emcid_embed_layernorm_f32(const float* tok, int64_t ld_tok, int64_t n_tok, const float* pos, int64_t ld_pos, int64_t n_pos,
                              const int64_t* token, const int* position, const float* gamma, const float* beta, float eps,
                              int64_t rows, int64_t cols, float* y, float* z, void* stream);

int64_t emcid_edit_workspace_bytes(int64_t N, int64_t d, int64_t h);

int emcid_edit_layer_f64(const float* K, const float* Zc, const float* zs_t, const float* C,
                         int64_t N, int64_t d, int64_t h,
                         double lam, double edit_weight, int layers_left,
                         const float* W0, float* W,
                         double* Xt_out, double* Rt_out, float* dW_out,
                         void* workspace, int64_t workspace_bytes, int* info_dev, void* stream);
int emcid_cov_inverse_f64(void* cov_factor_ws, int64_t n_layers, int64_t d, int64_t first_layer, int64_t count, void* stream);

int emcid_edit_layer_shard_f64(const float* K, const float* Zc, const float* zs_t, const float* C,
                               int64_t N, int64_t d, int64_t h, double lam, double edit_weight, int layers_left,
                               int64_t n_lo, int64_t n_hi, double* U_partial, double* Xt_out, double* Rt_out,
                               void* workspace, int64_t workspace_bytes, int* info_dev, void* stream);
int emcid_apply_update_f32(const double* U, const float* W0, float* W, float* dW, int64_t n, void* stream);

int64_t emcid_cov_factor_workspace_bytes(int64_t n_layers, int64_t d);
int emcid_factor_cov_f64(const float* const* C_host_list, int64_t n_layers, int64_t d, double lam, double edit_weight,
                         void* workspace, int64_t workspace_bytes, int* info_dev, void* stream);
int emcid_cov_factor_rescale_f64(const void* src_ws, void* dst_ws, int64_t workspace_bytes, int64_t n_layers, int64_t d, double a,
                                 int with_inverse, void* stream);
int64_t emcid_edit_dual_workspace_bytes(int64_t N, int64_t d, int64_t h);
enum {
    EMCID_DUAL_K = 0, EMCID_DUAL_P = 1, EMCID_DUAL_Y = 2, EMCID_DUAL_R = 3, EMCID_DUAL_S = 4, EMCID_DUAL_LS = 5,
    EMCID_DUAL_INVS = 6, EMCID_DUAL_PT = 7, EMCID_DUAL_Y2 = 8, EMCID_DUAL_V = 9, EMCID_DUAL_U = 10, EMCID_DUAL_SK = 11,
    EMCID_DUAL_XT = 12, EMCID_DUAL_TT = 13, EMCID_DUAL_SK_COUNTERS = 14
};
double* emcid_edit_dual_block(void* workspace, int64_t N, int64_t d, int64_t h, int which, int64_t* doubles_out);
enum { EMCID_SCHUR_XROW = 0, EMCID_SCHUR_FULL_INVERSE = 1, EMCID_SCHUR_SUBSTITUTION = 2 };
int emcid_edit_dual_schur_form(int64_t N, int64_t d, int64_t h);
int emcid_edit_dual_stage1_f64(const float* K, const float* Zc, const float* zs_t, int64_t N, int64_t d, int64_t h,
                               double edit_weight, int layers_left, double lam_ratio, const void* cov_factor_ws, int64_t n_layers,
                               int64_t layer_index, int64_t n_lo, int64_t n_hi, int use_inverse, void* workspace,
                               int64_t workspace_bytes, void* stream);
double* emcid_edit_dual_pt(void* workspace, int64_t N, int64_t d, int64_t h);
int emcid_edit_dual_stage2_f64(int64_t N, int64_t d, int64_t h, double lam_ratio, const float* W0, float* W, double* adjk_out, double* Rt_out,
                               float* dW_out, void* workspace, int64_t workspace_bytes, int* info_dev, void* stream);

int emcid_edit_dual_apply_stage1_f64(const float* K, const float* Zc, const float* zs_t, int64_t N, int64_t d, int64_t h,
                                     double edit_weight, int layers_left, double lam_ratio, const void* cov_factor_ws, int64_t n_layers,
                                     int64_t layer_index, int64_t n_lo, int64_t n_hi, int use_inverse, void* workspace,
                                     int64_t workspace_bytes, void* stream);
double* emcid_edit_dual_yt(void* workspace, int64_t N, int64_t d, int64_t h);
int emcid_edit_dual_apply_stage2_f64(int64_t N, int64_t d, int64_t h, const void* cov_factor_ws, int64_t n_layers,
                                     int64_t layer_index, int use_inverse, int assembled, const float* W0, float* W,
                                     float* dW_out, void* workspace, int64_t workspace_bytes, int* info_dev, void* stream);
int emcid_edit_dual_apply_assemble_f64(int64_t N, int64_t d, int64_t h, void* workspace, int64_t workspace_bytes, void* stream);

int64_t emcid_edit_dual_preserve_workspace_bytes(int64_t N, int64_t d, int64_t h, int64_t capacity);
int emcid_edit_layer_dual_preserve_f64(const float* K, const float* Zc, const float* zs_t, int64_t N, int64_t d, int64_t h,
                                       double edit_weight, int layers_left, double lam_ratio, const void* cov_factor_ws,
                                       int64_t n_layers, int64_t layer_index, double* Yp, int64_t ldy, double* Lp, int64_t ldl,
                                       double* tile_inv, int64_t capacity, int64_t M, const float* W0, float* W, float* dW_out,
                                       double* U_out, void* workspace, int64_t workspace_bytes, int* info_dev, void* stream);

int64_t emcid_session_retain_workspace_bytes(int64_t N, int64_t d, int64_t capacity);
int emcid_session_retain_f64(const float* K, int64_t N, int64_t d, double row_scale, double lam_ratio, const void* cov_factor_ws,
                             int64_t n_layers, int64_t layer_index, double* Yp, int64_t ldy, double* Lp, int64_t ldl,
                             double* tile_inv, int64_t capacity, int64_t M, void* workspace, int64_t workspace_bytes, int* info_dev,
                             void* stream);

int64_t emcid_session_release_workspace_bytes(int64_t n_rebuilt, int64_t d, int64_t capacity);
int emcid_session_release_f64(const int32_t* keep_dev, int64_t n_keep, int64_t first, int64_t d, double* Yp, int64_t ldy, double* Lp,
                              int64_t ldl, double* tile_inv, int64_t capacity, int64_t M, void* workspace, int64_t workspace_bytes,
                              int* info_dev, void* stream);

int emcid_session_step_norms_f64(const void* workspace, int64_t workspace_bytes, int64_t N, int64_t d, int64_t h, int64_t capacity,
                                 int64_t M, double* drift_out, double* left_out, double* resid_out, void* stream);

int64_t emcid_cov_factor_fold_workspace_bytes(int64_t M, int64_t d);
int emcid_cov_factor_fold_f64(const void* src_ws, double lam_ratio, const double* Yp, int64_t ldy, int64_t M, int64_t capacity,
                              const float* C, double lam, double edit_weight, int fill_base, void* dst_ws, int64_t n_layers,
                              int64_t d, int64_t layer_index, double* base, void* workspace, int64_t workspace_bytes,
                              int* info_dev, void* stream);

int emcid_session_refold_update_f64(void* cov_ws, int64_t n_layers, int64_t d, int64_t layer_index, const double* Yp, int64_t ldy,
                                    int64_t M, int64_t capacity, double* archive, int64_t lda, int64_t n_archived,
                                    const int32_t* rel_idx_dev, int64_t n_rel, double* base, void* stream);
int emcid_cov_factor_refactor_f64(void* cov_ws, int64_t workspace_bytes, int64_t n_layers, int64_t d, int* info_dev, void* stream);

int emcid_score_rows_f32(const float* a, int64_t lda, const float* b, int64_t ldb, const float* t, int64_t ldt, const float* gamma,
                         const float* beta, float eps, int64_t rows, int64_t cols, double* out, void* stream);
int emcid_score_chains_f64(const double* node, int64_t U, const int32_t* anc, int64_t ld_anc, const int32_t* depth,
                           const int64_t* end_node, int64_t B, double* out, void* stream);
int emcid_score_chains_pair_f64(const double* node1, int64_t U1, const int32_t* anc1, int64_t ld_anc1, const int32_t* depth1,
                                const int64_t* end1, const double* node2, int64_t U2, const int32_t* anc2, int64_t ld_anc2,
                                const int32_t* depth2, const int64_t* end2, int64_t B, double* out, void* stream);
int emcid_score_pooled_f32(const float* a, int64_t lda, const float* b, int64_t ldb, const float* gamma, const float* beta, float eps,
                           const float* P, int64_t ldp, int64_t rows, int64_t cols, int64_t proj, double* out, void* stream);

int64_t emcid_edit_lu_workspace_bytes(int64_t N, int64_t d, int64_t h);
int emcid_edit_layer_lu_f64(const float* K, const float* Zc, const float* zs_t, const float* C,
                            int64_t N, int64_t d, int64_t h, double lam, double edit_weight, int layers_left,
                            const float* W0, float* W, double* adjk_out, double* Rt_out, float* dW_out,
                            void* workspace, int64_t workspace_bytes, int* info_dev, void* stream);
int emcid_lu_solve_f64(double* A, int64_t lda, int64_t n, double* B, int64_t ldb, int64_t nrhs, int* piv_dev,
                       int* info_dev, void* stream);

int emcid_edit_dual_cols_stage1_f64(const float* K, const float* Zc, const float* zs_t, int64_t N, int64_t d, int64_t h,
                                    double edit_weight, int layers_left, double lam_ratio, const void* cov_factor_ws, int64_t n_layers,
                                    int64_t layer_index, const int* tiles_host, int n_tiles, void* workspace,
                                    int64_t workspace_bytes, void* stream);
double* emcid_edit_dual_s(void* workspace, int64_t N, int64_t d, int64_t h);
double* emcid_edit_dual_u(void* workspace, int64_t N, int64_t d, int64_t h);
int emcid_edit_dual_cols_stage2_f64(int64_t N, int64_t d, int64_t h, const void* cov_factor_ws, int64_t n_layers,
                                    int64_t layer_index, const int* tiles_host, int n_tiles, void* workspace,
                                    int64_t workspace_bytes, int* info_dev, void* stream);
int emcid_apply_update2d_f32(const double* U, int64_t ldu, const float* W0, float* W, float* dW, int64_t h, int64_t d,
                             void* stream);


int emcid_assemble_spd_f64(const float* C, int64_t ldc, const double* Kt64, int64_t Np, int64_t d, int64_t ldk,
                           double lam, float cw, double* A, int64_t lda, void* stream);
int64_t emcid_inverse_workspace_doubles(int64_t dp);
int emcid_debug_leaf_stamps(const double* A, double* L, double* inv, int* info_dev, long long* stamps_dev, void* stream);
int emcid_cholesky_f64(double* A, double* L, int64_t dp, int64_t lda, double* invdiag, int* info_dev, void* stream);
int emcid_cholesky_solve_f64(const double* L, int64_t dp, int64_t lda, const double* invdiag,
                             double* Bt, double* Yt, int64_t Np, int64_t ldb, void* stream);
int64_t emcid_full_inverse_scratch_doubles(int64_t dp, int64_t lda);
int emcid_full_inverse_f64(const double* L, int64_t dp, int64_t lda, const double* invdiag, double* X, double* scratch,
                           int64_t scratch_doubles, void* stream);
int emcid_delta_w_f64(const double* Rt, int64_t ldr, const double* Xt, int64_t ldx, int64_t Np, int64_t h, int64_t d,
                      const float* W0, float* W, int64_t ldw, float* dW, double* U, void* stream);

int emcid_dgemm_f64(int ta, int tb, int64_t M, int64_t N, int64_t K, double alpha,
                    const double* A, int64_t lda, const double* B, int64_t ldb,
                    double beta, double* C, int64_t ldc, void* stream);
int emcid_dgemm_ex_f64(int ta, int tb, int64_t M, int64_t N, int64_t K, double alpha,
                       const double* A, int64_t lda, const double* B, int64_t ldb,
                       double beta, double* C, int64_t ldc, int flags, int cfg, int ksplit, void* stream);

int64_t emcid_streamk_workspace_bytes(int wgs);
int emcid_dgemm_streamk_f64(int tb, int64_t M, int64_t N, int64_t K, double alpha, const double* A, int64_t lda,
                            const double* B, int64_t ldb, double* C, int64_t ldc, int flags, int wgs, double diag_add,
                            void* workspace, int64_t workspace_bytes, void* stream);

int emcid_debug_streamk_stamps(long long* stamps_dev);
int emcid_debug_step_stamps(long long* stamps_dev);

int emcid_dgemm_batched_f64(int ta, int tb, int64_t M, int64_t N, int64_t K, double alpha,
                            const double* A, int64_t lda, int64_t sA, const double* B, int64_t ldb, int64_t sB,
                            double beta, double* C, int64_t ldc, int64_t sC, int64_t batch, void* stream);

int emcid_axpy_f32(float* W, const float* dW, int64_t n, void* stream);

#ifdef __cplusplus
}
#endif
#endif
```

Baseline: 111,800.

## Add stream-K split-K path for sp16 linear GEMMs with partial-tile reduction

Adds a stream-K variant of the split-fp16 MFMA linear kernel. A fixed number of persistent workgroups (about two per CU) each cover a contiguous range of tile×K work, write partial accumulators to global slots, and the last arriver for each tile reduces them through atomic ticket counters. The aim is to remove wave-quantisation tail waste when the tile count is not a multiple of the CU slots. It needs a workspace and counter zeroing threaded through the CLIP layer calls and the Python wrapper, and the auto-selection looks gated off unless an environment flag or an explicit override enables it.

Result: slower. 110,200 (-1.5%).

```diff
diff --git a/emcid_amd/csrc/clip_layers.hip b/emcid_amd/csrc/clip_layers.hip
--- a/emcid_amd/csrc/clip_layers.hip
+++ b/emcid_amd/csrc/clip_layers.hip
@@ -1,4 +1,5 @@
 #include "common.h"
+#include "sp16.h"
 
 #include <algorithm>
 
@@ -95,11 +96,13 @@
     uint32_t* xq_p;
     float* xq_s;
     float* hs_q;
+    void* sk;
+    int64_t sk_bytes;
 };
 
 inline int64_t clip_ws_bytes(int64_t rows, int64_t h, int64_t d) {
     const int64_t r = round_up(rows, 64);
-    return 4 * (r * 3 * h + r * h + r * h + r + r * h + r + 2 * r + r * d + r * h + r + r * h) + 16 * 16;
+    return 4 * (r * 3 * h + r * h + r * h + r + r * h + r + 2 * r + r * d + r * h + r + r * h) + 16 * 16 + emcid_linear_sp16_workspace_size();
 }
 
 inline bool clip_ws_carve(void* base, int64_t bytes, int64_t rows, int64_t h, int64_t d, ClipWs& w) {
@@ -118,7 +121,14 @@
     w.xq_p = (uint32_t*)take(r * h);
     w.xq_s = (float*)take(r);
     w.hs_q = (float*)take(r * h);
+    w.sk_bytes = emcid_linear_sp16_workspace_size();
+    w.sk = w.sk_bytes > 0 ? take(w.sk_bytes / 4) : nullptr;
     return true;
+}
+
+inline bool clip_sk_wanted(int64_t rows, int64_t h, int64_t d, bool query_rows, int64_t n_sel) {
+    return query_rows ? (sp16_streamk_auto(rows, 2 * h, h) || sp16_streamk_auto(n_sel, h, h) || sp16_streamk_auto(n_sel, d, h))
+                      : (sp16_streamk_auto(rows, 3 * h, h) || sp16_streamk_auto(rows, d, h));
 }
 
 }
@@ -177,10 +187,10 @@
 
 int64_t emcid_clip_workspace_bytes(int64_t rows, int64_t h, int64_t d) { return clip_ws_bytes(rows, h, d); }
 
-int emcid_clip_layer_head_sp16(const emcid_clip_layer_sp16* L, int64_t rows, int64_t h, int64_t d, int64_t heads, float attn_scale,
-                               const int* anc, int64_t anc_ld, const int* depth, const int* rows_sel, int64_t n_sel,
-                               const float* hs, const void* x_planes, const float* x_inv_scale, float* mid, void* f_planes,
-                               float* f_scale, float* f_f32, void* workspace, int64_t workspace_bytes, void* stream) {
+static int clip_layer_head(const emcid_clip_layer_sp16* L, int64_t rows, int64_t h, int64_t d, int64_t heads, float attn_scale,
+                           const int* anc, int64_t anc_ld, const int* depth, const int* rows_sel, int64_t n_sel,
+                           const float* hs, const void* x_planes, const float* x_inv_scale, float* mid, void* f_planes,
+                           float* f_scale, float* f_f32, void* workspace, int64_t workspace_bytes, bool sk_zeroed, void* stream) {
     EMCID_CHECK_ARG(L && rows > 0 && h > 0 && d > 0 && heads > 0 && h % heads == 0 && anc && depth && hs && x_planes && x_inv_scale);
     EMCID_CHECK_ARG(mid && f_planes && f_scale && n_sel > 0 && n_sel <= rows && (rows_sel != nullptr || n_sel == rows) && h % 32 == 0 && d % 32 == 0);
     ClipWs w;
@@ -190,14 +200,15 @@
     const float* q;
     int64_t ldq;
     const float* res;
+    if (w.sk != nullptr && !sk_zeroed && clip_sk_wanted(rows, h, d, rows_sel != nullptr, n_sel)) EMCID_TRY(sp16_streamk_zero_counters(w.sk, st));
     if (rows_sel == nullptr) {
-        EMCID_TRY(emcid_linear_sp16_f32(x_planes, h, x_inv_scale, L->qkv_planes, h, L->qkv_inv_scale, L->qkv_bias, nullptr, 0, w.qkv,
-                                        3 * h, nullptr, 0, nullptr, rows, 3 * h, h, 0, -1, stream));
+        EMCID_TRY(emcid_linear_sp16_ws_f32(x_planes, h, x_inv_scale, L->qkv_planes, h, L->qkv_inv_scale, L->qkv_bias, nullptr, 0, w.qkv,
+                                           3 * h, nullptr, 0, nullptr, rows, 3 * h, h, 0, -1, w.sk, w.sk_bytes, 0, stream));
         q = w.qkv, ldq = 3 * h, res = hs;
     } else {
-        EMCID_TRY(emcid_linear_sp16_f32(x_planes, h, x_inv_scale, (const uint32_t*)L->qkv_planes + h * h, h, L->qkv_inv_scale + h,
-                                        L->qkv_bias ? L->qkv_bias + h : nullptr, nullptr, 0, w.qkv + h, 3 * h, nullptr, 0, nullptr,
-                                        rows, 2 * h, h, 0, -1, stream));
+        EMCID_TRY(emcid_linear_sp16_ws_f32(x_planes, h, x_inv_scale, (const uint32_t*)L->qkv_planes + h * h, h, L->qkv_inv_scale + h,
+                                           L->qkv_bias ? L->qkv_bias + h : nullptr, nullptr, 0, w.qkv + h, 3 * h, nullptr, 0, nullptr,
+                                           rows, 2 * h, h, 0, -1, w.sk, w.sk_bytes, 0, stream));
         {
             ScopedProf sp(KC_MISC, st);
             hipLaunchKernelGGL(gather_rows16_kernel, dim3((unsigned)n_sel), dim3(256), 0, st, (const unsigned char*)x_planes, 4 * h,
@@ -208,8 +219,8 @@
                                rows_sel, (unsigned char*)w.hs_q, 4 * h, (int)(4 * h));
             EMCID_CHECK_LAUNCH();
         }
-        EMCID_TRY(emcid_linear_sp16_f32(w.xq_p, h, w.xq_s, L->qkv_planes, h, L->qkv_inv_scale, L->qkv_bias, nullptr, 0, w.mid, h,
-                                        nullptr, 0, nullptr, n_sel, h, h, 0, -1, stream));
+        EMCID_TRY(emcid_linear_sp16_ws_f32(w.xq_p, h, w.xq_s, L->qkv_planes, h, L->qkv_inv_scale, L->qkv_bias, nullptr, 0, w.mid, h,
+                                           nullptr, 0, nullptr, n_sel, h, h, 0, -1, w.sk, w.sk_bytes, 0, stream));
         q = w.mid, ldq = h, res = w.hs_q;
     }
     EMCID_TRY(emcid_tree_attention_sp16(q, ldq, w.qkv + h, w.qkv + 2 * h, 3 * h, anc, anc_ld, depth, rows_sel, n_sel, heads, D,
@@ -218,9 +229,17 @@
                                     0, nullptr, n_sel, h, h, 0, -1, stream));
     EMCID_TRY(emcid_add_layernorm_sp16(mid, h, nullptr, 0, L->ln2_gamma, L->ln2_beta, L->ln2_eps, n_sel, h, nullptr, nullptr, w.z_p,
                                        h, w.z_s, L->fc1_bound, f_scale, stream));
-    EMCID_TRY(emcid_linear_sp16_f32(w.z_p, h, w.z_s, L->fc1_planes, h, L->fc1_inv_scale, L->fc1_bias, nullptr, 0, f_f32, d,
-                                    f_planes, d, f_scale, n_sel, d, h, L->act, -1, stream));
-    return EMCID_OK;
+    EMCID_TRY(emcid_linear_sp16_ws_f32(w.z_p, h, w.z_s, L->fc1_planes, h, L->fc1_inv_scale, L->fc1_bias, nullptr, 0, f_f32, d,
+                                       f_planes, d, f_scale, n_sel, d, h, L->act, -1, w.sk, w.sk_bytes, 0, stream));
+    return EMCID_OK;
+}
+
+int emcid_clip_layer_head_sp16(const emcid_clip_layer_sp16* L, int64_t rows, int64_t h, int64_t d, int64_t heads, float attn_scale,
+                               const int* anc, int64_t anc_ld, const int* depth, const int* rows_sel, int64_t n_sel,
+                               const float* hs, const void* x_planes, const float* x_inv_scale, float* mid, void* f_planes,
+                               float* f_scale, float* f_f32, void* workspace, int64_t workspace_bytes, void* stream) {
+    return clip_layer_head(L, rows, h, d, heads, attn_scale, anc, anc_ld, depth, rows_sel, n_sel, hs, x_planes, x_inv_scale, mid,
+                           f_planes, f_scale, f_f32, workspace, workspace_bytes, false, stream);
 }
 
 int emcid_clip_layer_tail_sp16(const emcid_clip_layer_sp16* L, int64_t n, int64_t h, int64_t d, const void* f_planes,
@@ -277,10 +296,13 @@
     EMCID_CHECK_ARG(layers && n_layers > 0 && hs && x_planes && x_inv_scale);
     ClipWs w;
     if (!clip_ws_carve(workspace, workspace_bytes, rows, h, d, w)) return fail(EMCID_ERR_BAD_ARG, __func__, "workspace too small or misaligned");
+    EMCID_CHECK_ARG(rows > 0 && h > 0 && d > 0);
+    const bool sk = w.sk != nullptr && clip_sk_wanted(rows, h, d, false, rows);
+    if (sk) EMCID_TRY(sp16_streamk_zero_counters(w.sk, (hipStream_t)stream));
     for (int64_t i = 0; i < n_layers; ++i) {
         const emcid_clip_layer_sp16* L = layers + i;
-        EMCID_TRY(emcid_clip_layer_head_sp16(L, rows, h, d, heads, attn_scale, anc, anc_ld, depth, nullptr, rows, hs, x_planes,
-                                             x_inv_scale, w.mid, w.f_p, w.f_scale, nullptr, workspace, workspace_bytes, stream));
+        EMCID_TRY(clip_layer_head(L, rows, h, d, heads, attn_scale, anc, anc_ld, depth, nullptr, rows, hs, x_planes, x_inv_scale, w.mid,
+                                  w.f_p, w.f_scale, nullptr, workspace, workspace_bytes, sk, stream));
         const bool last = i + 1 == n_layers;
         const float* g = last ? next_ln_gamma : layers[i + 1].ln1_gamma;
         const float* b = last ? next_ln_beta : layers[i + 1].ln1_beta;
diff --git a/emcid_amd/csrc/gemm_sp16.hip b/emcid_amd/csrc/gemm_sp16.hip
--- a/emcid_amd/csrc/gemm_sp16.hip
+++ b/emcid_amd/csrc/gemm_sp16.hip
@@ -1,7 +1,9 @@
 #include "common.h"
 #include "sp16.h"
+#include "sp16_streamk.h"
 
 #include <algorithm>
+#include <atomic>
 
 namespace emcid {
 
@@ -716,6 +718,119 @@
     }
 }
 
+struct SpStreamK {
+    float* partials;
+    unsigned* counters;
+    int slots;
+};
+
+constexpr int kSkSlotFloats = 128 * 128;
+
+template <int DBG>
+__global__ __launch_bounds__(256) __attribute__((amdgpu_waves_per_eu(2, 2))) void linear_sp16_streamk_kernel(SpArgs a, SpStreamK w) {
+    constexpr int MJ = 4, NI = 4, WM = 2, WN = 2, BM = 128, BN = 128, NT = 256;
+    constexpr int STAGE = (BM + BN) * 128, SIDE = 4 * (2 * BM + 2 * BN);
+    __shared__ __attribute__((aligned(1024))) unsigned char smem[2 * STAGE + SIDE + 16];
+    volatile int& s_last = *reinterpret_cast<volatile int*>(smem + 2 * STAGE + SIDE);
+    const int tid = threadIdx.x;
+    const SkPartition part = sk_partition(a.tiles, a.K / SPK, w.slots);
+    const int G = (int)gridDim.x;
+    int run = (int)blockIdx.x;
+    if (G % 8 == 0) run = (int)(blockIdx.x & 7) * (G / 8) + (int)(blockIdx.x >> 3);
+    if (run >= part.runs) return;
+    long long st_begin = 0, st_mark = 0, st_loop = 0, st_publish = 0, st_reduce = 0, st_epi = 0, st_segments = 0, st_clk = 0;
+    if constexpr (DBG == 2) {
+        st_begin = st_mark = (long long)__builtin_amdgcn_s_memrealtime();
+        st_clk = (long long)__builtin_amdgcn_s_memtime();
+    }
+    auto lap = [&](long long& sum) __attribute__((always_inline)) {
+        if constexpr (DBG == 2) {
+            const long long now = (long long)__builtin_amdgcn_s_memrealtime();
+            sum += now - st_mark;
+            st_mark = now;
+        }
+    };
+    long long u = sk_run_begin(part, run);
+    const long long u1 = sk_run_begin(part, run + 1);
+    float* side = reinterpret_cast<float*>(smem + 2 * STAGE);
+    while (u < u1) {
+        const SkSegment s = sk_segment_at(part, run, u);
+        int bm, bn;
+        sp_tile_of(a, s.tile, bm, bn);
+        const int m0 = bm * BM, n0 = bn * BN;
+        v4f acc[NI][MJ];
+        long long clk[2] = {0, 0};
+        SpSidePre<BM, BN, NT> pre{a, m0, n0, side};
+        sp_accumulate16<MJ, NI, WM, WN, 2, 0, true>(a.X + (int64_t)m0 * a.ldx + (int64_t)s.k_begin * SPK, a.ldx, a.M - m0,
+                                                    a.W + (int64_t)n0 * a.ldw + (int64_t)s.k_begin * SPK, a.ldw, a.N - n0,
+                                                    s.k_end - s.k_begin, smem, acc, pre, clk);
+        lap(st_loop);
+        ++st_segments;
+        bool finish = s.slot < 0;
+        if (!finish) {
+            const char* slot = reinterpret_cast<const char*>(w.partials + (int64_t)s.slot * kSkSlotFloats);
+            const unsigned lane_off = (unsigned)tid * 16u;
+#pragma unroll
+            for (int i = 0; i < NI; ++i)
+#pragma unroll
+                for (int j = 0; j < MJ; ++j) {
+                    const char* q = slot + (i * MJ + j) * NT * 16;
+                    const v4f x = acc[i][j];
+                    asm volatile("global_store_dwordx4 %0, %1, %2 sc1\n\ts_nop 1" ::"v"(lane_off), "v"(x), "s"(q) : "memory");
+                }
+            asm volatile("s_waitcnt vmcnt(0)" ::: "memory");
+            __syncthreads();
+            if (tid == 0) {
+                const unsigned old = __hip_atomic_fetch_add(w.counters + s.tile, 1u, __ATOMIC_RELAXED, __HIP_MEMORY_SCOPE_AGENT);
+                s_last = (old + 1 == (unsigned)sk_tickets(part, s.tile)) ? 1 : 0;
+            }
+            __syncthreads();
+            lap(st_publish);
+            if (__builtin_amdgcn_readfirstlane(s_last)) {
+#pragma unroll
+                for (int i = 0; i < NI; ++i)
+#pragma unroll
+                    for (int j = 0; j < MJ; ++j) acc[i][j] = (v4f){0.f, 0.f, 0.f, 0.f};
+                const int r_first = sk_first_run(part, s.tile), r_last = sk_last_run(part, s.tile);
+                for (int r = r_first; r <= r_last; ++r) {
+                    char* src = reinterpret_cast<char*>(w.partials + (int64_t)sk_slot_of(part, s.tile, r) * kSkSlotFloats);
+                    const __amdgpu_buffer_rsrc_t rs = __builtin_amdgcn_make_buffer_rsrc(src, 0, kSkSlotFloats * 4, 0x00020000);
+                    v4u raw[NI * MJ];
+#pragma unroll
+                    for (int v = 0; v < NI * MJ; ++v)
+                        raw[v] = __builtin_amdgcn_raw_buffer_load_b128(rs, (int)(tid * 16), v * NT * 16, 16 );
+                    __builtin_amdgcn_sched_barrier(0);
+#pragma unroll
+                    for (int i = 0; i < NI; ++i)
+#pragma unroll
+                        for (int j = 0; j < MJ; ++j) {
+                            const v4f x = __builtin_bit_cast(v4f, raw[i * MJ + j]);
+#pragma unroll
+                            for (int e = 0; e < 4; ++e) acc[i][j][e] += x[e];
+                        }
+                    __builtin_amdgcn_sched_barrier(0);
+                }
+                if (tid == 0) w.counters[s.tile] = 0;
+                finish = true;
+                lap(st_reduce);
+            }
+        }
+        if (finish) {
+            sp_finish16<MJ, NI, WM, WN>(a, m0, n0, smem, side, acc);
+            lap(st_epi);
+        }
+        u += s.k_end - s.k_begin;
+        __syncthreads();
+    }
+    if constexpr (DBG == 2) {
+        if (a.stamps != nullptr && tid == 0) {
+            long long* o = a.stamps + 8 * (int64_t)blockIdx.x;
+            o[0] = st_begin; o[1] = (long long)__builtin_amdgcn_s_memrealtime(); o[2] = st_loop; o[3] = st_publish; o[4] = st_reduce;
+            o[5] = st_epi; o[6] = st_segments; o[7] = (long long)__builtin_amdgcn_s_memtime() - st_clk;
+        }
+    }
+}
+
 __device__ __forceinline__ void sp_split8(const v4f& a, const v4f& b, float s, v4u& hi, v4u& lo) {
     v8h h, l;
 #pragma unroll
@@ -876,8 +991,46 @@
 }
 
 struct SpCfg { int bm, bn; };
-static const SpCfg kSpCfgs[] = {{128, 128}, {80, 128}, {64, 64}, {160, 128}, {64, 64}};
+static const SpCfg kSpCfgs[] = {{128, 128}, {80, 128}, {64, 64}, {160, 128}, {64, 64}, {128, 128}};
 inline long long* g_sp16_stamps = nullptr;
+static std::atomic<long long> g_sp16_paths[6];
+
+constexpr int kSkMaxTiles = 8192;
+constexpr int64_t kSkHead = 4096;
+
+static int sk_device_slots() {
+    static std::atomic<int> cache[64];
+    int dev = 0;
+    if (hipGetDevice(&dev) != hipSuccess || dev < 0 || dev >= 64) { (void)hipGetLastError(); return 0; }
+    int s = cache[dev].load(std::memory_order_relaxed);
+    if (s == 0) {
+        int cus = 0;
+        if (hipDeviceGetAttribute(&cus, hipDeviceAttributeMultiprocessorCount, dev) != hipSuccess) { (void)hipGetLastError(); return 0; }
+        s = 2 * cus / 8 * 8;
+        cache[dev].store(s, std::memory_order_relaxed);
+    }
+    return s;
+}
+
+constexpr double kSkMinWaste = 1.10;
+static bool sk_auto(int64_t M, int64_t N, int64_t K, int slots, bool overridden) {
+    static const int env = env_flag("EMCID_SP16_STREAMK", -1);
+    const int64_t tiles = ((M + 127) / 128) * ((N + 127) / 128);
+    if (env == 0 || (env < 0 && !overridden)) return false;
+    if (slots <= 0 || tiles < slots || tiles > kSkMaxTiles || K / SPK < 8) return false;
+    const int64_t rounds = (tiles + slots - 1) / slots;
+    return (double)(rounds * slots) >= kSkMinWaste * (double)tiles;
+}
+
+bool sp16_streamk_auto(int64_t M, int64_t N, int64_t K) {
+    const int64_t t128 = ((M + 127) / 128) * ((N + 127) / 128);
+    return t128 >= 400 && !(t128 >= 1600 && M >= 16384) && sk_auto(M, N, K, sk_device_slots(), false);
+}
+
+int sp16_streamk_zero_counters(void* workspace, hipStream_t st) {
+    char* counters = (char*)workspace + kSkHead + (int64_t)2 * sk_device_slots() * kSkSlotFloats * 4;
+    return hipMemsetAsync(counters, 0, (size_t)kSkMaxTiles * 4, st) == hipSuccess ? EMCID_OK : fail(EMCID_ERR_HIP, __func__, "hipMemsetAsync");
+}
 
 }
 
@@ -948,10 +1101,29 @@
     return EMCID_OK;
 }
 
+int64_t emcid_linear_sp16_workspace_size(void) {
+    const int slots = sk_device_slots();
+    return slots <= 0 ? 0 : kSkHead + (int64_t)2 * slots * kSkSlotFloats * 4 + (int64_t)kSkMaxTiles * 4;
+}
+
+int emcid_linear_sp16_path_counts(int64_t* counts6) {
+    EMCID_CHECK_ARG(counts6);
+    for (int i = 0; i < 6; ++i) counts6[i] = g_sp16_paths[i].load(std::memory_order_relaxed);
+    return EMCID_OK;
+}
+
 int emcid_linear_sp16_f32(const void* Xp, int64_t ldx, const float* x_inv_scale, const void* Wp, int64_t ldw,
                           const float* w_inv_scale, const float* bias, const float* residual, int64_t ldr, float* Y, int64_t ldy,
                           void* Yp, int64_t ldp, const float* y_scale, int64_t M, int64_t N, int64_t K, int act, int cfg,
                           void* stream) {
+    return emcid_linear_sp16_ws_f32(Xp, ldx, x_inv_scale, Wp, ldw, w_inv_scale, bias, residual, ldr, Y, ldy, Yp, ldp, y_scale, M, N, K,
+                                    act, cfg, nullptr, 0, 0, stream);
+}
+
+int emcid_linear_sp16_ws_f32(const void* Xp, int64_t ldx, const float* x_inv_scale, const void* Wp, int64_t ldw,
+                             const float* w_inv_scale, const float* bias, const float* residual, int64_t ldr, float* Y, int64_t ldy,
+                             void* Yp, int64_t ldp, const float* y_scale, int64_t M, int64_t N, int64_t K, int act, int cfg,
+                             void* workspace, int64_t workspace_bytes, int sk_slots, void* stream) {
     EMCID_CHECK_ARG(Xp && Wp && x_inv_scale && w_inv_scale && (Y || Yp) && M > 0 && N > 0 && K > 0 && ldx >= K && ldw >= K);
     EMCID_CHECK_ARG(K % SPK == 0 && ldx % 4 == 0 && ldw % 4 == 0 && aligned16(Xp) && aligned16(Wp));
     EMCID_CHECK_ARG(M < (1 << 24) && N < (1 << 24) && K < (1 << 24) && (residual == nullptr || ldr >= N) && (Y == nullptr || ldy >= N));
@@ -960,7 +1132,16 @@
     EMCID_CHECK_ARG(ldx < (1 << 20) && ldw < (1 << 20));
     const int dbg = cfg < 0 ? 0 : (cfg >> 4) & 3;
     int tile_sel = cfg < 0 ? -1 : (cfg & 15);
-    EMCID_CHECK_ARG(tile_sel <= 4 && (dbg == 0 || tile_sel == 0) && dbg != 2);
+    EMCID_CHECK_ARG(tile_sel <= 5 && (dbg == 0 || tile_sel == 0) && dbg != 2 && sk_slots >= 0);
+    EMCID_CHECK_ARG(workspace != nullptr || (tile_sel != 5 && workspace_bytes == 0));
+    int slots = 0;
+    if (workspace != nullptr) {
+        const int dev_slots = sk_device_slots();
+        EMCID_CHECK_ARG(aligned16(workspace) && dev_slots > 0 && sk_slots <= dev_slots);
+        EMCID_CHECK_WORKSPACE(workspace_bytes, emcid_linear_sp16_workspace_size(), " (see emcid_linear_sp16_workspace_size)");
+        slots = sk_slots > 0 ? sk_slots : dev_slots;
+    }
+    const bool auto_sel = tile_sel < 0;
     if (tile_sel < 0) {
         const int64_t t128 = ((M + 127) / 128) * ((N + 127) / 128), t80 = ((M + 79) / 80) * ((N + 127) / 128);
         const int64_t t64 = ((M + 63) / 64) * ((N + 63) / 64);
@@ -970,6 +1151,8 @@
         else if (t64 >= 256) tile_sel = 2;
         else tile_sel = 4;
     }
+    if (auto_sel && slots > 0 && residual == nullptr && (tile_sel == 0 || sk_slots > 0) && sk_auto(M, N, K, slots, sk_slots > 0)) tile_sel = 5;
+    if (tile_sel == 5 && (K / SPK < 2 || ((M + 127) / 128) * ((N + 127) / 128) > kSkMaxTiles)) tile_sel = 0;
     const int bm = kSpCfgs[tile_sel].bm, bn = kSpCfgs[tile_sel].bn;
     const int tiles_m = (int)((M + bm - 1) / bm), tiles_n = (int)((N + bn - 1) / bn);
     const int tiles = tiles_m * tiles_n;
@@ -979,6 +1162,16 @@
     const SpArgs a{(const uint32_t*)Xp, ldx, x_inv_scale, (const uint32_t*)Wp, ldw, w_inv_scale, bias, residual, ldr, Y, ldy,
                    (uint32_t*)Yp, ldp, y_scale, (int)M, (int)N, (int)K, act, tiles_n, tiles, rb, g_sp16_stamps};
     ScopedProf sp(KC_LINEAR, st);
+    g_sp16_paths[tile_sel].fetch_add(1, std::memory_order_relaxed);
+    if (tile_sel == 5) {
+        const SkPartition part = sk_partition(tiles, (int)(K / SPK), slots);
+        const SpStreamK w{reinterpret_cast<float*>((char*)workspace + kSkHead),
+                          reinterpret_cast<unsigned*>((char*)workspace + kSkHead + (int64_t)2 * sk_device_slots() * kSkSlotFloats * 4), slots};
+        if (a.stamps) hipLaunchKernelGGL((linear_sp16_streamk_kernel<2>), dim3((unsigned)part.runs), dim3(256), 0, st, a, w);
+        else hipLaunchKernelGGL((linear_sp16_streamk_kernel<0>), dim3((unsigned)part.runs), dim3(256), 0, st, a, w);
+        EMCID_CHECK_LAUNCH();
+        return EMCID_OK;
+    }
 #define EMCID_SP_DMA16(MJ_, NI_, WM_, WN_, NS_, WPE_, DBG_)                                                                        \
     hipLaunchKernelGGL((linear_sp16_dma16_kernel<MJ_, NI_, WM_, WN_, NS_, DBG_, WPE_>), dim3((unsigned)(per * 8)), dim3(64 * WM_ * WN_), 0, st, a)
     switch (tile_sel) {
diff --git a/emcid_amd/csrc/sp16.h b/emcid_amd/csrc/sp16.h
--- a/emcid_amd/csrc/sp16.h
+++ b/emcid_amd/csrc/sp16.h
@@ -26,4 +26,7 @@
     *reinterpret_cast<sp_v4h*>(dst + 16) = l;
 }
 
+bool sp16_streamk_auto(int64_t M, int64_t N, int64_t K);
+int sp16_streamk_zero_counters(void* workspace, hipStream_t st);
+
 }
diff --git a/emcid_amd/csrc/sp16_streamk.h b/emcid_amd/csrc/sp16_streamk.h
--- /dev/null
+++ b/emcid_amd/csrc/sp16_streamk.h
@@ -0,0 +1,53 @@
+#pragma once
+#include <stdint.h>
+
+#if defined(__HIPCC__) || defined(__CUDACC__)
+#define EMCID_SK_HD __host__ __device__ __forceinline__
+#else
+#define EMCID_SK_HD inline
+#endif
+
+namespace emcid {
+
+struct SkPartition {
+    int tiles, depth, runs;
+    long long total;
+};
+
+struct SkSegment {
+    int tile, k_begin, k_end;
+    int slot;
+};
+
+EMCID_SK_HD SkPartition sk_partition(int tiles, int depth, int slots) {
+    SkPartition p;
+    p.tiles = tiles, p.depth = depth, p.total = (long long)tiles * depth;
+    p.runs = (long long)slots < p.total ? slots : (int)p.total;
+    return p;
+}
+
+EMCID_SK_HD long long sk_run_begin(const SkPartition& p, int r) { return (long long)r * p.total / p.runs; }
+
+EMCID_SK_HD int sk_run_of(const SkPartition& p, long long u) { return (int)(((u + 1) * p.runs - 1) / p.total); }
+
+EMCID_SK_HD int sk_first_run(const SkPartition& p, int tile) { return sk_run_of(p, (long long)tile * p.depth); }
+EMCID_SK_HD int sk_last_run(const SkPartition& p, int tile) { return sk_run_of(p, (long long)(tile + 1) * p.depth - 1); }
+
+EMCID_SK_HD int sk_tickets(const SkPartition& p, int tile) { return sk_last_run(p, tile) - sk_first_run(p, tile) + 1; }
+
+EMCID_SK_HD SkSegment sk_segment_at(const SkPartition& p, int r, long long u) {
+    const long long u0 = sk_run_begin(p, r), u1 = sk_run_begin(p, r + 1);
+    SkSegment s;
+    s.tile = (int)(u / p.depth);
+    s.k_begin = (int)(u - (long long)s.tile * p.depth);
+    const long long left = u1 - u;
+    s.k_end = (long long)p.depth - s.k_begin < left ? p.depth : (int)(s.k_begin + left);
+    s.slot = (s.k_begin == 0 && s.k_end == p.depth) ? -1 : 2 * r + (u == u0 ? 0 : 1);
+    return s;
+}
+
+EMCID_SK_HD int sk_slot_of(const SkPartition& p, int tile, int r) {
+    return 2 * r + ((long long)tile * p.depth > sk_run_begin(p, r) ? 1 : 0);
+}
+
+}
diff --git a/emcid_amd/hip.py b/emcid_amd/hip.py
--- a/emcid_amd/hip.py
+++ b/emcid_amd/hip.py
@@ -32,7 +32,7 @@
     "emcid_edit_lu_workspace_bytes", "emcid_edit_layer_lu_f64", "emcid_lu_solve_f64",
     "emcid_edit_dual_cols_stage1_f64", "emcid_edit_dual_s", "emcid_edit_dual_u", "emcid_edit_dual_cols_stage2_f64",
     "emcid_apply_update2d_f32", "emcid_linear_f32", "emcid_linear_ws_f32", "emcid_linear_workspace_bytes",
-    "emcid_split_rows_f16", "emcid_linear_sp16_f32", "emcid_gram_sp16_workspace_bytes", "emcid_gram_sp16_workspace_bytes_for", "emcid_gram_accumulate_sp16_f32", "emcid_add_layernorm_sp16", "emcid_embed_layernorm_sp16",
+    "emcid_split_rows_f16", "emcid_linear_sp16_f32", "emcid_linear_sp16_ws_f32", "emcid_linear_sp16_workspace_size", "emcid_linear_sp16_path_counts", "emcid_gram_sp16_workspace_bytes", "emcid_gram_sp16_workspace_bytes_for", "emcid_gram_accumulate_sp16_f32", "emcid_add_layernorm_sp16", "emcid_embed_layernorm_sp16",
     "emcid_tree_attention_sp16", "emcid_tree_attention_sp16_supported", "emcid_clip_workspace_bytes",
     "emcid_clip_layer_head_sp16", "emcid_clip_layer_tail_sp16", "emcid_clip_layers_sp16", "emcid_clip_edit_layer_tail_sp16",
     "emcid_edit_dual_block", "emcid_edit_dual_schur_form", "emcid_full_inverse_scratch_doubles", "emcid_full_inverse_f64",
@@ -152,6 +152,9 @@
                                                  p, p, p, p, p, p, p, p, i64, p, p, i64, p, p, p, f32, p, p, p]),
         "emcid_tree_attention_sp16": (i32, [p, i64, p, p, i64, p, i64, p, p, i64, i64, i64, f32, p, i64, p, p]),
         "emcid_linear_sp16_f32": (i32, [p, i64, p, p, i64, p, p, p, i64, p, i64, p, i64, p, i64, i64, i64, i32, i32, p]),
+        "emcid_linear_sp16_ws_f32": (i32, [p, i64, p, p, i64, p, p, p, i64, p, i64, p, i64, p, i64, i64, i64, i32, i32, p, i64, i32, p]),
+        "emcid_linear_sp16_workspace_size": (i64, []),
+        "emcid_linear_sp16_path_counts": (i32, [p]),
         "emcid_add_layernorm_f32": (i32, [p, i64, p, i64, p, p, C.c_float, i64, i64, p, p, p]),
         "emcid_embed_layernorm_f32": (i32, [p, i64, i64, p, i64, i64, p, p, p, p, C.c_float, i64, i64, p, p, p]),
         "emcid_tree_attention_f32": (i32, [p, i64, p, p, i64, p, i64, p, p, i64, i64, i64, f32, p, i64, p]),
@@ -574,7 +577,9 @@
     if ws is None:
         if len(_LINEAR_WS) >= 8:
             _LINEAR_WS.clear()
-        ws = _LINEAR_WS[key] = torch.zeros(int(load().emcid_linear_workspace_bytes()), dtype=torch.uint8, device=dev)
+        with torch.cuda.device(dev):
+            nbytes = max(int(load().emcid_linear_workspace_bytes()), int(load().emcid_linear_sp16_workspace_size()))
+        ws = _LINEAR_WS[key] = torch.zeros(nbytes, dtype=torch.uint8, device=dev)
     return ws
 
 
@@ -663,7 +668,7 @@
 
 def linear_sp(x: SplitRows, w: SplitRows, bias: Optional[torch.Tensor] = None, act: int = ACT_NONE,
               residual: Optional[torch.Tensor] = None, out: Optional[torch.Tensor] = None, want_f32: bool = True,
-              planes_scale: Optional[torch.Tensor] = None, cfg: int = -1):
+              planes_scale: Optional[torch.Tensor] = None, cfg: int = -1, sk_slots: int = 0):
     M, K = x.planes.shape
     N = w.planes.shape[0]
     if w.planes.shape[1] != K or K % 32:
@@ -689,15 +694,31 @@
     if LINEAR_FLOPS["count"]:
         LINEAR_FLOPS["flops"] += 2.0 * M * N * K
         LINEAR_FLOPS["launches"] += 1
-    _check(load().emcid_linear_sp16_f32(
-        _ptr(x.planes), x.planes.stride(0), _ptr(x.inv_scale, torch.float32, "x scale"), _ptr(w.planes), w.planes.stride(0),
-        _ptr(w.inv_scale, torch.float32, "w scale"), _ptr(bias, torch.float32, "bias"), _ptr(residual, torch.float32, "residual"),
-        residual.stride(0) if residual is not None else 0, _ptr(y), y.stride(0) if y is not None else 0, _ptr(yp),
-        yp.stride(0) if yp is not None else 0, _ptr(planes_scale, torch.float32, "planes scale"), M, N, K, int(act), int(cfg),
-        _stream(x.planes)), "emcid_linear_sp16_f32")
+    ws = None
+    if (cfg < 0 or (cfg & 15) == 5) and not torch.cuda.is_current_stream_capturing():
+        ws = _linear_workspace(dev)
+    try:
+        _check(load().emcid_linear_sp16_ws_f32(
+            _ptr(x.planes), x.planes.stride(0), _ptr(x.inv_scale, torch.float32, "x scale"), _ptr(w.planes), w.planes.stride(0),
+            _ptr(w.inv_scale, torch.float32, "w scale"), _ptr(bias, torch.float32, "bias"), _ptr(residual, torch.float32, "residual"),
+            residual.stride(0) if residual is not None else 0, _ptr(y), y.stride(0) if y is not None else 0, _ptr(yp),
+            yp.stride(0) if yp is not None else 0, _ptr(planes_scale, torch.float32, "planes scale"), M, N, K, int(act), int(cfg),
+            C.c_void_p(ws.data_ptr()) if ws is not None else None, ws.numel() if ws is not None else 0, int(sk_slots),
+            _stream(x.planes)), "emcid_linear_sp16_ws_f32")
+    except EmcidHipError:
+        if ws is not None:
+            _LINEAR_WS.pop((dev.index if dev.index is not None else torch.cuda.current_device(),
+                            torch.cuda.current_stream(dev).cuda_stream), None)
+        raise
     if planes_scale is None:
         return y
     return SplitRows(yp, planes_scale[1], y)
+
+
+def linear_sp_path_counts() -> list:
+    out = (C.c_int64 * 6)()
+    _check(load().emcid_linear_sp16_path_counts(out), "emcid_linear_sp16_path_counts")
+    return list(out)
 
 
 def add_layernorm(a: torch.Tensor, b: Optional[torch.Tensor], ln: torch.nn.LayerNorm, want_sum: bool = True):
diff --git a/include/emcid_hip.h b/include/emcid_hip.h
--- a/include/emcid_hip.h
+++ b/include/emcid_hip.h
@@ -54,6 +54,13 @@
                           const float* w_inv_scale, const float* bias, const float* residual, int64_t ldr, float* Y, int64_t ldy,
                           void* Yp, int64_t ldp, const float* y_scale, int64_t M, int64_t N, int64_t K, int act, int cfg,
                           void* stream);
+
+int64_t emcid_linear_sp16_workspace_size(void);
+int emcid_linear_sp16_ws_f32(const void* Xp, int64_t ldx, const float* x_inv_scale, const void* Wp, int64_t ldw,
+                             const float* w_inv_scale, const float* bias, const float* residual, int64_t ldr, float* Y, int64_t ldy,
+                             void* Yp, int64_t ldp, const float* y_scale, int64_t M, int64_t N, int64_t K, int act, int cfg,
+                             void* workspace, int64_t workspace_bytes, int sk_slots, void* stream);
+int emcid_linear_sp16_path_counts(int64_t* counts6);
 
 int emcid_debug_linear_sp16_stamps(long long* stamps_dev);
 int64_t emcid_gram_sp16_workspace_bytes(int64_t d);
```
